# statsleelab/gauss

Measured on AMD Instinct MI355X. Metric: imputed SNPs/sec (whole node) at 1/2/4/8 GPUs; LD-GEMM MFMA TFLOP/s vs peak, higher is better.
Workload: dtype f32

## Files before the change

### gauss_amd/_lib.py

```python
import ctypes as C
import os

import numpy as np

_HERE = os.path.dirname(os.path.abspath(__file__))
LIB_PATH = os.path.join(_HERE, "lib", "libgauss_hip.so")

MODE_POOLED = 0
MODE_WEIGHTED = 1
ST_CLAMPED = 1
ST_NONFINITE = 2
ST_NOCONV = 4
WIN_IMPUTE = 0
WIN_QCAT = 1
WIN_LD = 2
GENO_U8, GENO_2BIT = 0, 1
SLCT_MAX = 32
TRAITS_MORE_MAX = 63
ST_SLCT_SKIPPED = 8
CODE_ADDITIVE, CODE_DOMINANT, CODE_RECESSIVE = 1, 2, 4
GRAM_F32 = 0
GRAM_I8 = 1

_dp = C.POINTER(C.c_double)
_ip = C.POINTER(C.c_int32)
_u8p = C.c_void_p


class WindowDesc(C.Structure):
    _fields_ = [
        ("mode", C.c_int), ("n_pop", C.c_int), ("pop_off", _ip), ("pop_wgt", _dp),
        ("n_measured", C.c_int), ("n_unmeasured", C.c_int),
        ("geno_m", _u8p), ("geno_u", _u8p), ("ld", C.c_int64), ("z1", _dp),
        ("lambda_", C.c_double), ("min_abs_eig", C.c_double),
        ("out_z", _dp), ("out_info", _dp), ("out_status", _ip), ("out_b11", _dp), ("out_b21", _dp),
        ("kind", C.c_int), ("n_head_measured", C.c_int), ("n_pred_measured", C.c_int), ("eig_cutoff", C.c_double),
        ("out_r", _dp), ("out_num_eig", _ip), ("u_codings", C.c_int),
        ("geno_format", C.c_int), ("rows_m", _ip), ("rows_u", _ip), ("pop_src_off", _ip),
        ("slct_max", C.c_int), ("slct_chi2_stop", C.c_double), ("slct_min_var_frac", C.c_double),
        ("slct_forced", _ip), ("n_slct_forced", C.c_int), ("out_slct_n", _ip), ("out_slct_idx", _ip),
        ("out_slct_zin", _dp), ("out_slct_joint", _dp), ("out_slct_zc", _dp), ("out_slct_var", _dp),
        ("n_traits_more", C.c_int), ("z_more", _dp), ("out_z_more", _dp),
        ("out_loo_z", _dp), ("out_loo_info", _dp), ("out_loo_t", _dp),
    ]


class GaussHipError(RuntimeError):
    pass


_lib = None

SYMBOLS = [
    "gauss_hip_init", "gauss_hip_device_count", "gauss_hip_device_of", "gauss_hip_destroy", "gauss_last_error", "gauss_hip_version", "gauss_hip_set_gram_dtype", "gauss_pinned_alloc", "gauss_pinned_free", "gauss_store_upload", "gauss_store_free", "gauss_pack2bit_device", "gauss_ld", "gauss_ld_per_pop", "gauss_ld_per_pop_pairs",
    "gauss_impute_window", "gauss_gene_ld_batch", "gauss_gram_counts", "gauss_job_create",
    "gauss_ld_rows", "gauss_gene_ld_batch_rows", "gauss_job_run", "gauss_job_fetch", "gauss_job_destroy", "gauss_job_span_ms", "gauss_job_profile",
    "gauss_job_profile_get", "gauss_job_work", "gauss_job_stats", "gauss_synth_device",
    "gauss_store_upload_async", "gauss_store_upload_fd_async", "gauss_store_wait", "gauss_store_alloc", "gauss_store_fill", "gauss_store_fill_fd", "gauss_store_upload_fd", "gauss_hip_context_id", "gauss_hip_add_destroy_hook", "gauss_hip_trim_cache", "gauss_hip_source_hash", "gauss_hip_counters", "gauss_job_counters", "gauss_hip_queues",
    "gauss_pop_weights", "gauss_zmix_normal_eq", "gauss_ld_resampled_rows",
]


def load():
    global _lib
    if _lib is not None:
        return _lib
    if not os.path.exists(LIB_PATH):
        raise GaussHipError(
            f"{LIB_PATH} not found: build it with `python -m gauss_amd.build` "
            "(gauss_amd has no CPU fallback by design)")
    lib = C.CDLL(LIB_PATH)
    for name in SYMBOLS:
        if not hasattr(lib, name):
            raise GaussHipError(f"libgauss_hip.so does not export {name}")
    lib.gauss_last_error.restype = C.c_char_p
    lib.gauss_hip_version.restype = C.c_char_p
    lib.gauss_hip_source_hash.restype = C.c_char_p
    lib.gauss_hip_init.argtypes = [C.c_int, C.POINTER(C.c_void_p)]
    lib.gauss_hip_device_count.argtypes = [C.POINTER(C.c_int)]
    lib.gauss_hip_device_of.argtypes = [C.c_void_p]
    lib.gauss_hip_destroy.argtypes = [C.c_void_p]
    lib.gauss_hip_destroy.restype = None
    lib.gauss_hip_set_gram_dtype.argtypes = [C.c_void_p, C.c_int]
    lib.gauss_pinned_alloc.argtypes = [C.c_void_p, C.c_int64, C.POINTER(C.c_void_p)]
    lib.gauss_pinned_free.argtypes = [C.c_void_p, C.c_void_p]
    lib.gauss_store_upload.argtypes = [C.c_void_p, C.c_void_p, C.c_int64, C.POINTER(C.c_void_p)]
    lib.gauss_store_free.argtypes = [C.c_void_p, C.c_void_p]
    lib.gauss_store_upload_async.argtypes = [C.c_void_p, C.c_void_p, C.c_int64, C.POINTER(C.c_void_p)]
    lib.gauss_store_wait.argtypes = [C.c_void_p, C.c_void_p, C.c_int64]
    lib.gauss_store_alloc.argtypes = [C.c_void_p, C.c_int64, C.POINTER(C.c_void_p)]
    lib.gauss_store_fill.argtypes = [C.c_void_p, C.c_void_p, C.c_void_p, C.c_int64, C.c_int64]
    lib.gauss_store_fill_fd.argtypes = [C.c_void_p, C.c_void_p, C.c_int, C.c_int64, C.c_int64, C.c_int64]
    lib.gauss_store_upload_fd.argtypes = [C.c_void_p, C.c_int, C.c_int64, C.c_int64, C.POINTER(C.c_void_p)]
    lib.gauss_ld.argtypes = [C.c_void_p, C.c_int, _u8p, C.c_int, C.c_int64, _ip, _dp, C.c_int,
                             C.c_double, _dp]
    lib.gauss_pack2bit_device.argtypes = [C.c_void_p, C.c_void_p, C.c_int64, C.c_void_p, C.c_int64, C.c_int, _ip, C.c_int]
    lib.gauss_ld_per_pop.argtypes = [C.c_void_p, _u8p, C.c_int, C.c_int64, _ip, C.c_int, _dp]
    lib.gauss_ld_per_pop_pairs.argtypes = [C.c_void_p, _u8p, C.c_int, C.c_int64, _ip, C.c_int, _ip, C.c_int, _ip, _ip, C.c_int64, _dp]
    lib.gauss_impute_window.argtypes = [C.c_void_p, C.POINTER(WindowDesc)]
    lib.gauss_gene_ld_batch.argtypes = [C.c_void_p, C.c_int, _u8p, C.c_int, C.c_int64, _ip, _dp,
                                        C.c_int, _ip, C.c_int, C.c_double, _dp]
    lib.gauss_ld_rows.argtypes = [C.c_void_p, C.c_int, _u8p, C.c_int64, C.c_int, _ip, C.c_int, _ip, _ip, _dp, C.c_int, C.c_double,
                                  C.c_int, _dp]
    lib.gauss_gene_ld_batch_rows.argtypes = [C.c_void_p, C.c_int, _u8p, C.c_int64, C.c_int, _ip, C.c_int, _ip, _ip, _dp, C.c_int,
                                             _ip, C.c_int, C.c_double, C.c_int, _dp]
    lib.gauss_gram_counts.argtypes = [C.c_void_p, _u8p, C.c_int, C.c_int, C.c_int64,
                                      C.POINTER(C.c_int64)]
    lib.gauss_job_create.argtypes = [C.c_void_p, C.POINTER(WindowDesc), C.c_int, C.c_int,
                                     C.POINTER(C.c_void_p)]
    lib.gauss_job_run.argtypes = [C.c_void_p]
    lib.gauss_job_fetch.argtypes = [C.c_void_p]
    lib.gauss_job_destroy.argtypes = [C.c_void_p]
    lib.gauss_job_destroy.restype = None
    lib.gauss_job_span_ms.argtypes = [C.c_void_p, C.c_void_p, _dp]
    lib.gauss_job_profile.argtypes = [C.c_void_p, C.c_int]
    lib.gauss_job_profile_get.argtypes = [C.c_void_p, C.c_int, _dp, C.POINTER(C.c_int64)]
    lib.gauss_job_counters.argtypes = [C.c_void_p, C.POINTER(C.c_int64)]
    lib.gauss_job_work.argtypes = [C.c_void_p, _dp, _dp, _dp, C.POINTER(C.c_int64)]
    lib.gauss_job_stats.argtypes = [C.c_void_p, _dp]
    lib.gauss_hip_context_id.argtypes = [C.c_void_p]
    lib.gauss_hip_context_id.restype = C.c_uint64
    lib.gauss_hip_trim_cache.argtypes = [C.c_void_p, C.POINTER(C.c_int64)]
    lib.gauss_hip_counters.argtypes = [C.c_void_p, C.POINTER(C.c_int64)]
    lib.gauss_hip_queues.argtypes = [C.c_void_p, C.POINTER(C.c_int32)]
    lib.gauss_synth_device.argtypes = [C.c_void_p, C.c_void_p, C.c_int, C.c_int64, _ip, C.c_int,
                                       C.POINTER(C.c_float), C.POINTER(C.c_float), C.c_uint64]
    lib.gauss_pop_weights.argtypes = [C.c_void_p, _dp, C.POINTER(C.c_int64), C.c_int, C.c_int, C.c_double, _dp, _ip]
    lib.gauss_zmix_normal_eq.argtypes = [C.c_void_p, _u8p, C.c_int, C.c_int64, _ip, C.c_int, _ip, C.c_int, _dp, _dp, _dp, _dp,
                                         C.POINTER(C.c_int64)]
    lib.gauss_ld_resampled_rows.argtypes = [C.c_void_p, _u8p, C.c_int64, C.c_int, _ip, C.c_int, _ip, _ip, C.c_int, _ip, _ip, C.c_int64,
                                            C.c_int64, C.c_double, C.c_int, _dp]
    _lib = lib
    return lib


def check(rc):
    if rc != 0:
        raise GaussHipError(f"gauss_hip error {rc}: {load().gauss_last_error().decode()}")


def as_u8(g):
    g = np.ascontiguousarray(g)
    if g.dtype != np.uint8:
        g = g.astype(np.uint8)
    return g


def ptr(a, t):
    return a.ctypes.data_as(t) if a is not None else None
```

### gauss_amd/csrc/gauss_abi.cpp

```cpp
#include "gauss_job.h"

#define JOB_ALIVE(job)                                                                                          \
    do {                                                                                                        \
        if (!(job)) return fail(GAUSS_E_INVALID, "job is NULL");                                                \
        if (!(job)->ctx) return fail(GAUSS_E_INVALID, "the job's context has been destroyed (gauss_hip_destroy)"); \
    } while (0)

static WinSpec spec_from_desc(const gauss_window_desc& d)
{
    WinSpec w;
    w.mode = d.mode; w.n_pop = d.n_pop; w.pop_off = d.pop_off; w.pop_wgt = d.pop_wgt;
    w.M = d.n_measured; w.U = d.n_unmeasured; w.geno_m = d.geno_m; w.geno_u = d.geno_u; w.ld = d.ld;
    w.z1 = d.z1; w.lambda = d.lambda; w.eps = d.min_abs_eig; w.diag = 1.0; w.ld_only = 0;
    w.gene_off = nullptr; w.n_gene = 0;
    w.kind = d.kind; w.n_head = d.n_head_measured; w.n_predm = d.n_pred_measured; w.eig_cutoff = d.eig_cutoff;
    w.u_codings = d.u_codings;
    w.geno_fmt = d.geno_format; w.rows_m = d.rows_m; w.rows_u = d.rows_u; w.pop_src_off = d.pop_src_off;
    w.out_b11 = d.out_b11; w.out_b21 = d.out_b21;
    w.out_loo_z = d.out_loo_z; w.out_loo_info = d.out_loo_info; w.out_loo_t = d.out_loo_t;
    w.n_traits_more = d.n_traits_more; w.z_more = d.z_more; w.out_z_more = d.out_z_more;
    w.slct_max = d.slct_max; w.slct_chi2_stop = d.slct_chi2_stop; w.slct_min_var_frac = d.slct_min_var_frac;
    w.slct_forced = d.slct_forced; w.n_slct_forced = d.n_slct_forced;
    w.out_slct_n = d.out_slct_n; w.out_slct_idx = d.out_slct_idx; w.out_slct_zin = d.out_slct_zin;
    w.out_slct_joint = d.out_slct_joint; w.out_slct_zc = d.out_slct_zc; w.out_slct_var = d.out_slct_var;
// ... 2 lines not shown
extern "C" {

int gauss_job_create(gauss_ctx* ctx, const gauss_window_desc* wins, int n_win, int on_device, gauss_job** out_job)
{
    if (!ctx || !wins || n_win < 1 || !out_job) return fail(GAUSS_E_INVALID, "bad arguments to gauss_job_create");
    std::vector<WinSpec> specs;
    for (int i = 0; i < n_win; i++) {
        if (wins[i].n_unmeasured < 1 && wins[i].kind != GAUSS_WIN_LD &&
            !(wins[i].kind == GAUSS_WIN_QCAT && wins[i].n_pred_measured > 0))
            return fail(GAUSS_E_INVALID, "window %d has no unmeasured SNPs", i);
        specs.push_back(spec_from_desc(wins[i]));
    }
    gauss_job* job = nullptr;
    int rc = job_build(ctx, specs, on_device, &job);
    if (rc) return rc;
    for (int i = 0; i < n_win; i++) {
        Plan& pl = job->plans[i];
        pl.out_z = wins[i].out_z; pl.out_info = wins[i].out_info; pl.out_status = wins[i].out_status;
        pl.out_b11 = wins[i].out_b11; pl.out_b21 = wins[i].out_b21;
        pl.out_r = wins[i].out_r; pl.out_num_eig = wins[i].out_num_eig;
    }
    *out_job = job;
    return GAUSS_OK;
}

int gauss_job_run(gauss_job* job) { JOB_ALIVE(job); return job_run(job, true); }
int gauss_job_fetch(gauss_job* job) { JOB_ALIVE(job); return job_fetch(job); }
void gauss_job_destroy(gauss_job* job) { job_free(job); }

int gauss_job_span_ms(gauss_job* first, gauss_job* last, double* out_ms)
{
    JOB_ALIVE(first); JOB_ALIVE(last);
    if (!out_ms || !first->ran || !last->ran) return fail(GAUSS_E_INVALID, "gauss_job_span_ms: both jobs must have run");
    HIPCHK(hipEventSynchronize(last->done));
    float ms = 0.f;
    HIPCHK(hipEventElapsedTime(&ms, first->begin, last->done));
    *out_ms = (double)ms;
    return GAUSS_OK;
}

int gauss_job_profile(gauss_job* job, int enable)
{
    JOB_ALIVE(job);
    if (job->prof && !enable) prof_collect(job);
    job->prof = enable != 0;
    if (enable) { for (int k = 0; k < 5; k++) { job->prof_ms[k] = 0; job->prof_n[k] = 0; } }
    return GAUSS_OK;
}

int gauss_job_profile_get(gauss_job* job, int kernel, double* out_ms, int64_t* out_launches)
{
    JOB_ALIVE(job);
    if (kernel < 0 || kernel > 4) return fail(GAUSS_E_INVALID, "bad arguments");
    hipStreamSynchronize(job->ctx->stream);
    prof_collect(job);
    if (out_ms) *out_ms = job->prof_ms[kernel];
    if (out_launches) *out_launches = job->prof_n[kernel];
    return GAUSS_OK;
}

int gauss_job_work(gauss_job* job, double* out_ld_flops, double* out_solve_flops, double* out_bytes, int64_t* out_imputed)
{
    if (!job) return fail(GAUSS_E_INVALID, "job is NULL");
    double ldf = 0, sf = 0, by = 0;
    int64_t imp = 0;
    for (const Plan& pl : job->plans) {
        const double M = pl.p.M, U = pl.p.U, N = pl.p.N;
        ldf += N * M * (M + 1) + 2.0 * N * U * M;
        sf += M * M * M / 3.0 + 2.0 * U * M * M + 4.0 * U * M;
        by += (M + U) * N + (M * M + U * M) * 8.0;
        imp += pl.p.U;
    }
    if (out_ld_flops) *out_ld_flops = ldf;
    if (out_solve_flops) *out_solve_flops = sf;
    if (out_bytes) *out_bytes = by;
    if (out_imputed) *out_imputed = imp;
    return GAUSS_OK;
}

int gauss_job_counters(gauss_job* job, int64_t* out4)
{
    if (!job || !out4) return fail(GAUSS_E_INVALID, "bad arguments to gauss_job_counters");
    out4[0] = job->n_merged; out4[1] = job->n_demoted; out4[2] = job->n_giveups; out4[3] = job->n_rerun_failed;
    return GAUSS_OK;
}

int gauss_job_stats(gauss_job* job, double* out4)
{
    if (!job || !out4) return fail(GAUSS_E_INVALID, "bad arguments");
    double flops = 0, slab = 0;
    const bool shm = job->gplan != nullptr;
    const bool edge16 = true;
    auto add = [&](const Plan& pl, bool skip_b11) {
        const Prob& p = pl.p;
        const int mt = p.Mp / TILE;
        auto rows = [&](int t) {
            if (!pl.tile_live.empty()) return pl.tile_live[(size_t)t];
            int left = (t < mt) ? p.M - t * TILE : p.U - (t - mt) * TILE; return left > TILE ? TILE : left;
        };
        auto halves = [](int r, int w) { int n = (r - w * 64 + 31) / 32; return n < 0 ? 0 : (n > 2 ? 2 : n); };
        double k_main = 0;
        {
            const int gran = job->gram_i8 ? 32 : 8;
            const std::vector<int>& blk = (p.geno_fmt == GAUSS_GENO_2BIT && !pl.run_pk_off.empty()) ? pl.run_pk_off : pl.pop_pk_off;
            const bool runs = &blk == &pl.run_pk_off;
            for (size_t q = 0; q + 1 < blk.size(); q++) {
                int live = blk[q + 1] - blk[q];
                if (!runs && q + 1 < pl.pop_raw_off.size()) live = pl.pop_raw_off[q + 1] - pl.pop_raw_off[q];
                else if (runs && pl.run_len_known(q)) live = pl.run_len[q];
                k_main += (double)((live + gran - 1) / gran * gran);
            }
        }
        const bool packed = job->gram_packed && p.slab16;
        int pairs = 0;
        for (int pr = 0; pr < p.npair; pr++) {
            const int ti = pl.pair_ti[pr], tj = pl.pair_tj[pr];
            if (skip_b11 && ti < mt) continue;
            pairs++;
            double tiles32 = 0, tiles_edge = 0;
            for (int wr = 0; wr < 2; wr++)
                for (int wc = 0; wc < 2; wc++) {
                    if (ti == tj && wr == 1 && wc == 0) continue;
                    int na = halves(rows(ti), wr);
                    if (packed && na > 1) na = 1;
                    int nb16 = (rows(tj) - wc * 64 + 15) / 16;
                    nb16 = nb16 < 0 ? 0 : (nb16 > 4 ? 4 : nb16);
                    if (edge16 && !job->gram_i8 && na > 0 && (nb16 & 1)) { tiles_edge += na * nb16 * 0.5; continue; }
                    double t32 = na * halves(rows(tj), wc);
                    if (ti == tj && wr == wc && t32 == 4) t32 = 3;
                    tiles32 += t32;
                }
            flops += 32.0 * 32.0 * 2.0 * (tiles32 * k_main + tiles_edge * p.Kp);
        }
        slab += (double)pairs * p.nseg * TILE * TILE * (p.slab16 ? sizeof(uint16_t) : sizeof(float));
    };
    for (const Plan& pl : job->plans) add(pl, shm);
    if (shm) add(*job->gplan, false);
    out4[0] = job->n_items; out4[1] = flops; out4[2] = slab; out4[3] = (double)job->ws_bytes;
    return GAUSS_OK;
}

int gauss_impute_window(gauss_ctx* ctx, const gauss_window_desc* win)
{
    if (!ctx || !win) return fail(GAUSS_E_INVALID, "bad arguments to gauss_impute_window");
    const bool fused = env_int("GAUSS_FUSED_SOLVE", 1) != 0;
    bool streamed = env_int("GAUSS_STREAM_WINDOW", 1) != 0 && fused && !win->rows_m && !win->rows_u && win->n_unmeasured >= 1 &&
                    win->n_measured >= 1 && win->kind != GAUSS_WIN_LD && (win->u_codings & ~GAUSS_CODE_ADDITIVE) == 0 &&
                    win->geno_m && win->geno_u && win->pop_off && win->n_pop >= 1 && win->n_pop <= 64;
    size_t row_bytes = 0;
    if (streamed) {
        const int N = win->pop_off[win->n_pop];
        if (win->geno_format == GAUSS_GENO_U8) {
            streamed = N >= 1 && win->ld >= N;
            row_bytes = (size_t)std::max(N, 0);
        } else if (win->geno_format == GAUSS_GENO_2BIT && win->ld % 16 == 0) {
            long long end = 0;
            for (int q = 0; q < win->n_pop && streamed; q++) {
                const long long blk = (long long)rup((size_t)std::max(win->pop_off[q + 1] - win->pop_off[q], 0), 64) / 4;
                const long long off = win->pop_src_off ? win->pop_src_off[q] : end;
                if (off < 0 || off % 16 || off + blk > win->ld) streamed = false;
                if (!win->pop_src_off) end = off + blk;
                row_bytes = std::max(row_bytes, (size_t)(off + blk));
            }
        } else streamed = false;
    }
    gauss_job* job = nullptr;
// ... 382 lines not shown
```

### gauss_amd/csrc/gauss_ctx.cpp

```cpp
#include "gauss_job.h"

thread_local std::string g_err;

int fail(int code, const char* fmt, ...)
{
    char buf[512];
    va_list ap;
    va_start(ap, fmt);
    vsnprintf(buf, sizeof(buf), fmt, ap);
    va_end(ap);
    g_err = buf;
    return code;
}

bool trace_on(const char* what)
{
    const char* e = getenv("GAUSS_TRACE");
    if (!e || !*e) return false;
    return strstr(e, "all") != nullptr || strstr(e, what) != nullptr;
}

static std::mutex g_hook_mu;
static std::vector<std::pair<void (*)(gauss_ctx*, uint64_t, void*), void*>> g_destroy_hooks;
static std::atomic<uint64_t> g_next_ctx_id{1};
// ... 105 lines not shown
static void ctx_flush_dev_cache_locked(gauss_ctx* c)
{
    for (auto& kv : c->dev_cache.free_blocks) { (void)hipFree(kv.second); c->block_size.erase(kv.second); }
    c->dev_cache.free_blocks.clear(); c->dev_cache.held = 0;
    (void)hipGetLastError();
}
hipError_t ctx_malloc_retry(gauss_ctx* c, void** out, size_t bytes)
{
    hipError_t e = hipMalloc(out, bytes);
    if (e == hipSuccess) return e;
    {
        std::lock_guard<std::mutex> lock(c->mu);
        if (c->dev_cache.free_blocks.empty()) return e;
        ctx_flush_dev_cache_locked(c);
    }
    return hipMalloc(out, bytes);
}

hipError_t ctx_dev_alloc(gauss_ctx* c, size_t bytes, void** out)
{
    std::lock_guard<std::mutex> lock(c->mu);
    if (void* p = c->dev_cache.take(bytes)) { *out = p; return hipSuccess; }
    hipError_t e = hipMalloc(out, bytes);
    if (e != hipSuccess && !c->dev_cache.free_blocks.empty()) {
        ctx_flush_dev_cache_locked(c);
        e = hipMalloc(out, bytes);
    }
    if (e == hipSuccess) c->block_size[*out] = bytes;
    return e;
}
void ctx_dev_release(gauss_ctx* c, void* p)
{
    if (!p) return;
    std::lock_guard<std::mutex> lock(c->mu);
    auto it = c->block_size.find(p);
    const size_t bytes = it == c->block_size.end() ? 0 : it->second;
    if (bytes && c->dev_cache.held + bytes <= c->dev_cache_limit) { c->dev_cache.free_blocks.emplace(bytes, p); c->dev_cache.held += bytes; return; }
    if (it != c->block_size.end()) c->block_size.erase(it);
    (void)hipFree(p);
}
hipError_t ctx_pin_alloc(gauss_ctx* c, size_t bytes, void** out)
{
    std::lock_guard<std::mutex> lock(c->mu);
    if (void* p = c->pin_cache.take(bytes)) { *out = p; return hipSuccess; }
    hipError_t e = hipHostMalloc(out, bytes, hipHostMallocDefault);
    if (e == hipSuccess) c->block_size[*out] = bytes;
    return e;
}
void ctx_pin_release(gauss_ctx* c, void* p)
{
    if (!p) return;
    std::lock_guard<std::mutex> lock(c->mu);
    auto it = c->block_size.find(p);
    const size_t bytes = it == c->block_size.end() ? 0 : it->second;
    if (bytes && c->pin_cache.held + bytes <= PIN_CACHE_LIMIT) { c->pin_cache.free_blocks.emplace(bytes, p); c->pin_cache.held += bytes; return; }
    if (it != c->block_size.end()) c->block_size.erase(it);
    (void)hipHostFree(p);
}

extern "C" {

const char* gauss_last_error(void) { return g_err.c_str(); }
const char* gauss_hip_version(void) { return "gauss_hip 0.2 (gfx950)"; }

int gauss_hip_init(int device, gauss_ctx** out_ctx)
{
    if (!out_ctx) return fail(GAUSS_E_INVALID, "out_ctx is NULL");
    int n = 0;
    HIPCHK(hipGetDeviceCount(&n));
    if (device < 0 || device >= n) return fail(GAUSS_E_INVALID, "device %d out of range (have %d)", device, n);
    HIPCHK(hipSetDevice(device));
    std::unique_ptr<gauss_ctx> guard(new gauss_ctx());
    gauss_ctx* c = guard.get();
    c->device = device;
    c->id = g_next_ctx_id.fetch_add(1);
    {
        size_t free_b = 0, total_b = 0;
        if (hipMemGetInfo(&free_b, &total_b) != hipSuccess) { total_b = (size_t)288 << 30; (void)hipGetLastError(); }
        c->dev_cache_limit = total_b / 3;
    }
    const char* e = getenv("GAUSS_GRAM_DTYPE");
    c->gram_i8 = (e && (strcmp(e, "i8") == 0 || strcmp(e, "int8") == 0)) ? 1 : 0;
    c->gram_packed = env_int("GAUSS_GRAM_PACKED", 1) != 0 ? 1 : 0;
    const char* one = getenv("GAUSS_SIDE_STREAM");
    c->main_cls = (one && atoi(one) == 0) ? STREAM_NORMAL : STREAM_HIGH;
    int rc = ctx_stream_create(c, &c->stream, c->main_cls);
    if (!rc && c->main_cls == STREAM_HIGH) {
        rc = ctx_stream_create(c, &c->side, STREAM_LOW);
        if (!rc) rc = ctx_stream_create(c, &c->chain, STREAM_HIGH);
    }
    if (!rc) rc = ctx_stream_create(c, &c->upload, STREAM_HIGH);
    if (rc) {
        ctx_stream_destroy(c, &c->upload, STREAM_HIGH);
        ctx_stream_destroy(c, &c->chain, STREAM_HIGH);
        ctx_stream_destroy(c, &c->side, STREAM_LOW);
        ctx_stream_destroy(c, &c->stream, c->main_cls);
        return rc;
    }
    if (c->chain && c->side) c->queues_probed_distinct = queues_side_by_side(c, c->chain, c->stream) && queues_side_by_side(c, c->side, c->stream);
    c->prepin = std::thread([c]() {
        (void)hipSetDevice(c->device);
        {
            void* d = nullptr;
            if (hipMalloc(&d, 256) == hipSuccess) {
                (void)hipMemsetAsync(d, 0, 256, c->upload);
                (void)hipStreamSynchronize(c->upload);
                (void)hipFree(d);
            } else (void)hipGetLastError();
        }
        for (int b = 0; b < 2; b++) {
            void* p = nullptr;
            if (hipHostMalloc(&p, UPLOAD_CHUNK, hipHostMallocDefault) != hipSuccess) { (void)hipGetLastError(); break; }
            { std::lock_guard<std::mutex> lock(c->mu); c->block_size[p] = UPLOAD_CHUNK; }
            ctx_pin_release(c, p);
        }
    });
    { QueueRegistry& r = registry(); std::lock_guard<std::mutex> lock(r.count_mu); r.ctxs.push_back(c); }
    *out_ctx = guard.release();
    return GAUSS_OK;
}

int gauss_hip_device_count(int* out_n)
{
    if (!out_n) return fail(GAUSS_E_INVALID, "out_n is NULL");
    int n = 0;
    hipError_t e = hipGetDeviceCount(&n);
    if (e == hipErrorNoDevice) { n = 0; e = hipSuccess; (void)hipGetLastError(); }
    if (e != hipSuccess) return fail(GAUSS_E_DEVICE, "hipGetDeviceCount failed: %s", hipGetErrorString(e));
    *out_n = n;
    return GAUSS_OK;
}

int gauss_hip_device_of(const gauss_ctx* ctx) { return ctx ? ctx->device : fail(GAUSS_E_INVALID, "ctx is NULL"); }


void gauss_hip_destroy(gauss_ctx* ctx)
{
    if (!ctx) return;
    hipSetDevice(ctx->device);
    ctx_join_prepin(ctx);
    std::vector<std::pair<void (*)(gauss_ctx*, uint64_t, void*), void*>> hooks;
    { std::lock_guard<std::mutex> lock(g_hook_mu); hooks = g_destroy_hooks; }
    for (auto& h : hooks) h.first(ctx, ctx->id, h.second);
    std::vector<gauss_job*> live;
    { std::lock_guard<std::mutex> lock(ctx->mu); live.assign(ctx->jobs.begin(), ctx->jobs.end()); }
    for (gauss_job* j : live) job_release(j);
    hipStreamSynchronize(ctx->stream);
    {
        QueueRegistry& r = registry();
        std::unique_lock<std::shared_mutex> excl(r.mu);
        { std::lock_guard<std::mutex> lock(r.count_mu); r.ctxs.erase(std::remove(r.ctxs.begin(), r.ctxs.end(), ctx), r.ctxs.end()); }
        ctx_stream_destroy(ctx, &ctx->side, STREAM_LOW);
        delete ctx->worker;
        ctx_stream_destroy(ctx, &ctx->copy, STREAM_NORMAL);
        ctx_stream_destroy(ctx, &ctx->aux, STREAM_HIGH);
        ctx_stream_destroy(ctx, &ctx->chain, STREAM_HIGH);
    }
    for (hipEvent_t e : ctx->ev_pool) hipEventDestroy(e);
    if (ctx->landing) (void)hipFree(ctx->landing);
    for (auto& kv : ctx->uploads) kv.second->finish();
    ctx->uploads.clear();
    ctx_stream_destroy(ctx, &ctx->upload, STREAM_HIGH);
    for (auto& kv : ctx->stores) (void)hipFree(const_cast<void*>(kv.first));
    ctx->stores.clear();
    for (auto& kv : ctx->dev_cache.free_blocks) (void)hipFree(kv.second);
    for (auto& kv : ctx->pin_cache.free_blocks) (void)hipHostFree(kv.second);
// ... 78 lines not shown
```

### gauss_amd/csrc/gauss_internal.h

```cpp
#pragma once
#include <hip/hip_runtime.h>
#include <stdint.h>
#include <atomic>
#include <mutex>

namespace gauss {

constexpr int TILE = 128;
constexpr int KC = 64;
constexpr int SEG_MAX = 2048;
constexpr int NB = 64;
constexpr int NR = 64;
constexpr int NRU = NR - 1;
constexpr int WIN_QCAT = 1;
constexpr int WIN_LD = 2;
constexpr int TILE_GB11 = 1 << 30;

#if defined(__HIP_DEVICE_COMPILE__)
#define GP(T) T __attribute__((address_space(1)))*
#else
#define GP(T) T*
#endif

struct Prob {
    int mode, P;
    int M, U;
    int Mp, Up, Sp;
    int N;
    int Kp;
    int nseg, npair, nT;
    int Mld, nblk;
    int npanel;
    int npi;
    int Up128;
    int ld_only;
    int kind;
    int n_head, n_predm;
    int n_rhs;
    int U_raw;
    int code_blk[3];
    int n_run;
    int geno_fmt;
    int gram_i8;
    int slab16;
    double lambda, eps, diag;
    long long ld_raw;
    GP(const uint8_t) raw_m;
    GP(const uint8_t) raw_u;
    GP(uint8_t) packed;
    GP(uint8_t) packed_u;
    GP(int) sx;
    GP(int) sxx;
    GP(int) sx_u;
    GP(int) sxx_u;
    GP(const int) pop_raw_off;
    GP(const int) pop_pk_off;
    GP(const double) pop_w;
    GP(const double) pop_wf;
    GP(const double) pop_md;
    GP(const int) seg_pop;
    GP(const int) seg_k0;
    GP(const int) seg_k1;
    GP(const int) pop_seg0;
    GP(const int) pair_ti;
    GP(const int) pair_tj;
    GP(const int) pair_lut;
    GP(const uint8_t) word_pop;
    GP(const int) rows_m;
    GP(const int) rows_u;
    GP(const uint8_t) word_run;
    GP(const int) run_pk_off;
    GP(const int) run_src;
    GP(float) slab;
    GP(double) rt_sd;
    GP(double) rt_wm;
    GP(double) rt_mu;
    GP(double) rt_wmu;
    GP(double) rt_sd_u;
    GP(double) rt_wm_u;
    GP(double) rt_mu_u;
    GP(double) rt_wmu_u;
    int g0;
    int n_gpair;
    GP(const int) gpair_ti;
    GP(const int) gpair_tj;
    GP(float) slab_g;
    GP(const double) z1;
    GP(double) A;
    GP(double) Linv;
    GP(double) B21;
    GP(double) V;
    GP(double) Gsum;
    GP(double) Part;
    GP(double) out_z;
    GP(double) out_info;
    GP(int) status;
    GP(double) out_ld;
    GP(const int) gene_off;
    int n_gene;
    GP(long long) gene_out_off;
    GP(const int) draw_col;
    int row_src_bytes;
    GP(double) out_loo;
    int slct_max, n_slct_forced;
    double slct_chi2_stop, slct_min_var_frac;
    GP(const int) slct_forced;
    GP(double) slct_W;
    GP(double) out_slct;
    int traits_T;
    GP(const double) traits_Z;
    GP(double) traits_Y;
    GP(double) traits_G;
    GP(double) out_traits;
};
constexpr int TRAITS_MAX = 63;
constexpr int traits_t16(int T) { return (T + 15) & ~15; }
constexpr int SLCT_K = 32;
constexpr int SLCT_T = 512;
constexpr int SLCT_M_MAX = 64 * SLCT_T;
constexpr size_t slct_doubles(int M, int K) { return 2 * (size_t)M + 3 * (size_t)K + 2; }

struct Item {
    GP(const uint8_t) a;
    GP(const uint8_t) b;
    GP(float) slab;
    GP(const int) seg_k1;
    GP(const uint32_t) chunk_live;
    int Kp;
    int k0;
    int nseg;
    int rows_a, rows_b;
    int flags;
};
static_assert(sizeof(Item) == 64, "work items are fetched as one 64-byte descriptor");

template <typename T> using gptr = T __attribute__((address_space(1)))*;
template <typename T> __device__ __forceinline__ gptr<T> G(T* p) { return (gptr<T>)p; }
template <typename T> __device__ __forceinline__ gptr<T> G(gptr<T> p) { return p; }

#if defined(__HIPCC__)
template <typename T>
__device__ __forceinline__ T uniform_load(GP(const T) p, int idx)
{
    return ((const T __attribute__((address_space(4)))*)p)[idx];
}
__device__ __forceinline__ int chunk_live_units(uint32_t word, int chunk)
{
    const int n = (int)((word >> (4 * (chunk & 7))) & 15u);
    return n ? n : 8;
}
#endif

struct DeviceOnce {
    std::atomic<unsigned long long> done{0};
    std::mutex mu;
    template <typename F> void run(F&& set)
    {
        int d = 0;
        (void)hipGetDevice(&d);
        const unsigned long long bit = 1ull << (d & 63);
        if (done.load(std::memory_order_acquire) & bit) return;
        std::lock_guard<std::mutex> lock(mu);
        if (done.load(std::memory_order_relaxed) & bit) return;
        set();
        done.fetch_or(bit, std::memory_order_release);
    }
};

void launch_pack_stats(const Prob* d_probs, const int2* d_rowmap, int n_rows, hipStream_t s);
constexpr int SIMLD_LDS_MAX = 60 << 10;
int resample_pack_lds_bytes(long long row_src_bytes);
void launch_resample_pack(const Prob* d_probs, const int2* d_rowmap, int n_rows, int lds_bytes, hipStream_t s);
void launch_gram(const Item* d_items, int n_items, int dtype_i8, hipStream_t s, unsigned long long* d_b11_done = nullptr);
void launch_wait_count(const unsigned long long* d_count, unsigned long long target, int* d_status, int n_status, hipStream_t s,
                       double bound_us = 0.0);
void launch_wait_count_for(const unsigned long long* d_count, unsigned long long target, int* d_status, hipStream_t s, double bound_us);
void launch_count_up(unsigned long long* d_count, hipStream_t s);
void launch_epilogue(const Prob* d_probs, const int2* d_tilemap, int n_tiles, int max_pop, int dtype_i8, hipStream_t s);
void launch_epilogue_b11_lite(const Prob* d_probs, const int2* d_tilemap, int n_tiles, int dtype_i8, hipStream_t s);
void launch_pop_cor(const Prob* d_probs, int prob, int npair, double* d_out, hipStream_t s);
void launch_zmix_normal_eq(const Prob* d_probs, int prob, int npair, const int* d_pop_group, int n_group, const double* d_z,
                           double* d_part, long long* d_part_n, double* d_out, long long* d_out_n, hipStream_t s);
void launch_pair_cor(const Prob* d_probs, int prob, const int2* d_pairs, long long n_pairs, const int* d_pop_group, int n_group,
                     double* d_out, hipStream_t s);
void launch_gene_epilogue(const Prob* d_probs, int prob, int n_gene, hipStream_t s);
void launch_factor_step(const Prob* d_probs, int n_prob, int step, int max_nblk, int max_npanel, int split, int own_panel, hipStream_t s);
void launch_factor_step_lite(const Prob* d_probs, int n_prob, int step, int max_nblk, int max_npanel, int split, hipStream_t s);
void launch_solve_last_lite(const Prob* d_probs, const int2* d_panelmap, int n_panels, int max_nblk, int split, hipStream_t s);
void launch_shift_cert(const Prob* d_probs, int n_prob, hipStream_t s);
void launch_solve(const Prob* d_probs, const int2* d_panelmap, int n_panels, hipStream_t s);
void launch_impute_gemm(const Prob* d_probs, const int2* d_gmap, int n_tiles, int u_tile, const int2* d_fmap, int n_chunks, hipStream_t s);
void launch_solve_last(const Prob* d_probs, const int2* d_panelmap, int n_panels, int max_nblk, int split, hipStream_t s);
void launch_loo(const Prob* d_probs, const int2* d_loomap, int n_panels, hipStream_t s);
void launch_slct(const Prob* d_probs, const int* d_slctmap, int n, hipStream_t s);
void launch_traits_weights(const Prob* d_probs, const int2* d_map, int n_blocks, hipStream_t s);
void launch_traits_impute(const Prob* d_probs, const int2* d_umap, int n_strips, hipStream_t s);
void launch_counts(const Prob* d_probs, int prob, int npair, long long* d_out, hipStream_t s);
void launch_pack2bit(const uint8_t* d_in, long long ld_in, uint8_t* d_out, long long ld_out, int n_snp,
                     const int* d_pop_off, const int* d_blk_off, int n_pop, hipStream_t s);
void launch_h2d_copy(void* d_dst, const void* pinned_src, size_t bytes, hipStream_t s);
struct ExportD {
    const double* src;
    double* dst;
    int rows, width, pitch, pad_;
};
void launch_export_rows(const ExportD* d_exports, int n, long long max_elems, hipStream_t s);
struct PwChunk { long long r0, r1; int iv, pad_; };
void launch_pop_weights(const double* d_x, int n_pop, const PwChunk* d_chunks, int n_chunk, const int* d_chunk_off,
                        const long long* d_off, int n_interval, double eps, double* d_part1, double* d_mean, double* d_part2,
                        double* d_w, int* d_status, hipStream_t s);
void launch_synth(uint8_t* d_out, int n_snp, long long ld, const int* d_pop_off, int n_pop,
                  int n_samples, const float* d_thr, const float* d_rho, uint64_t seed,
                  hipStream_t s);

}
```

### gauss_amd/csrc/gauss_job.h

```cpp
#pragma once
#include "gauss_internal.h"
#pragma GCC visibility push(default)
#include "../../include/gauss_hip.h"
#pragma GCC visibility pop

#include <algorithm>
#include <atomic>
#include <chrono>
#include <condition_variable>
#include <cmath>
#include <cstdarg>
#include <cstdio>
#include <cstring>
#include <deque>
#include <functional>
#include <map>
#include <memory>
#include <mutex>
#include <set>
#include <shared_mutex>
#include <thread>
#include <string>
#include <vector>

// ... 33 lines not shown

struct CopyWorker {
    std::mutex mu;
    std::condition_variable cv;
    std::function<void()> task;
    bool busy = false, stop = false;
    std::thread th;
    explicit CopyWorker(int device)
    {
        th = std::thread([this, device]() {
            (void)hipSetDevice(device);
            std::unique_lock<std::mutex> lock(mu);
            for (;;) {
                cv.wait(lock, [&] { return stop || task; });
                if (stop) return;
                std::function<void()> t;
                t.swap(task);
                lock.unlock();
                t();
                lock.lock();
                busy = false;
                cv.notify_all();
            }
        });
    }
    void submit(std::function<void()> t)
    {
        std::lock_guard<std::mutex> lock(mu);
        task = std::move(t); busy = true;
        cv.notify_all();
    }
    void wait()
    {
        std::unique_lock<std::mutex> lock(mu);
        cv.wait(lock, [&] { return !busy; });
    }
    ~CopyWorker()
    {
        { std::lock_guard<std::mutex> lock(mu); stop = true; cv.notify_all(); }
        if (th.joinable()) th.join();
    }
};

struct StoreUpload {
    void* d = nullptr;
    size_t bytes = 0;
    std::thread th;
    std::mutex mu;
    std::condition_variable cv;
    std::vector<std::pair<size_t, hipEvent_t>> marks;
    bool done = false;
    int rc = 0;
    std::string err;
    std::mutex join_mu;
    void finish() { std::lock_guard<std::mutex> lock(join_mu); if (th.joinable()) th.join(); }
    ~StoreUpload()
    {
        finish();
        for (auto& m : marks) if (m.second) hipEventDestroy(m.second);
    }
};

enum StreamClass { STREAM_NORMAL = 0, STREAM_HIGH = 1, STREAM_LOW = 2 };

struct gauss_ctx {
    int device;
    uint64_t id = 0;
    hipStream_t stream = nullptr;
    StreamClass main_cls = STREAM_HIGH;
    hipStream_t side = nullptr;
    hipStream_t copy = nullptr;
    hipStream_t aux = nullptr;
    hipStream_t chain = nullptr;
    struct CopyWorker* worker = nullptr;
    uint8_t* landing = nullptr;
    size_t landing_bytes = 0;
    std::vector<hipEvent_t> ev_pool;
    std::mutex stream_mu;
    std::mutex run_mu;
    hipStream_t upload = nullptr;
    std::map<const void*, std::shared_ptr<StoreUpload>> uploads;
    int gram_i8 = 0;
    int gram_packed = 1;
    std::map<const void*, size_t> stores;
    std::mutex mu;
    BlockCache dev_cache, pin_cache;
    std::map<void*, size_t> block_size;
    std::set<gauss_job*> jobs;
    size_t dev_cache_limit = 0;
    std::thread prepin;
    std::mutex prepin_mu;
    int n_hi = 0, n_lo = 0;
    bool queues_probed_distinct = false;
    std::atomic<long long> n_runs_merged{0}, n_runs_demoted{0}, n_merged_giveups{0}, n_rerun_failed{0};
};

int ctx_stream_create(gauss_ctx* c, hipStream_t* out, StreamClass cls);
void ctx_stream_destroy(gauss_ctx* c, hipStream_t* s, StreamClass cls);
std::shared_mutex& queue_registry_mutex();
bool queues_exclusive(int device);
void ctx_join_prepin(gauss_ctx* c);

hipError_t ctx_malloc_retry(gauss_ctx* c, void** out, size_t bytes);
hipError_t ctx_dev_alloc(gauss_ctx* c, size_t bytes, void** out);
void ctx_dev_release(gauss_ctx* c, void* p);
hipError_t ctx_pin_alloc(gauss_ctx* c, size_t bytes, void** out);
void ctx_pin_release(gauss_ctx* c, void* p);

bool trace_on(const char* what);

constexpr double GRAM_PACKED_COST = 0.58;
static inline int env_int(const char* name, int dflt) { const char* e = getenv(name); return e ? atoi(e) : dflt; }

constexpr int GEMM_SMALL_TILES = 1600;
constexpr int OWN_PANEL_MAX_WINDOWS = 20;
constexpr int SOLVE_SPLIT_MIN = 2;

static const size_t PIN_CACHE_LIMIT = (size_t)1 << 30;
static const size_t UPLOAD_CHUNK = (size_t)32 << 20;
static inline size_t rup(size_t x, size_t a) { return (x + a - 1) / a * a; }

struct DevBuf {
    void* p = nullptr;
    DevBuf() = default;
    DevBuf(const DevBuf&) = delete;
    DevBuf& operator=(const DevBuf&) = delete;
    ~DevBuf() { if (p) (void)hipFree(p); }
    hipError_t alloc(size_t bytes) { return hipMalloc(&p, bytes ? bytes : 1); }
    hipError_t alloc(gauss_ctx* c, size_t bytes) { return ctx_malloc_retry(c, &p, bytes ? bytes : 1); }
    template <typename T> T* as() const { return (T*)p; }
};
struct Plan {
    Prob p;
    std::vector<int> pop_raw_off, pop_pk_off, seg_pop, seg_k0, seg_k1, pop_seg0;
    std::vector<int> pair_ti, pair_tj, pair_lut;
    std::vector<double> pop_w, pop_wf, pop_md, z1;
    std::vector<uint8_t> word_pop, word_run;
    std::vector<uint32_t> chunk_live;
    std::vector<int> run_pk_off, run_src, run_len;
    bool run_len_known(size_t q) const { return q < run_len.size(); }
    std::vector<int32_t> rows_m, rows_u;
    std::vector<int32_t> draw_col;
    size_t row_bytes = 0;
    std::vector<int> gene_off;
    std::vector<long long> gene_out_off;
    std::vector<std::pair<int, int>> groups;
    std::vector<std::pair<int, int>> fine;
    std::vector<int> tile_live;
    const uint8_t* h_geno_m = nullptr;
    const uint8_t* h_geno_u = nullptr;
    long long user_ld = 0;
    double* out_z = nullptr;
    double* out_info = nullptr;
    int32_t* out_status = nullptr;
    double* out_b11 = nullptr;
    double* out_b21 = nullptr;
    double* out_r = nullptr;
    int32_t* out_num_eig = nullptr;
    bool loo = false;
    double* out_loo_z = nullptr;
    double* out_loo_info = nullptr;
    double* out_loo_t = nullptr;
    int slct_K = 0;
    std::vector<int> slct_forced;
    int32_t* out_slct_n = nullptr;
    int32_t* out_slct_idx = nullptr;
    double* out_slct_zin = nullptr;
    double* out_slct_joint = nullptr;
    double* out_slct_zc = nullptr;
    double* out_slct_var = nullptr;
    int traits_T = 0;
    std::vector<double> traits_z;
    double* out_z_more = nullptr;
    size_t res_count() const
    { return 2 * (size_t)p.n_rhs + (loo ? 3 * (size_t)p.M : 0) + (size_t)traits_T * p.U + (slct_K ? slct_doubles(p.M, slct_K) : 0); }
    double* out_ld_user = nullptr;
    int U_user = 0;
    size_t out_ld_count = 0;
    double* d_b11_copy = nullptr;
    size_t res_off = 0;
};

struct ProfSlot { hipEvent_t a, b; int kernel; unsigned run; int launches = 1; };

struct gauss_job {
    gauss_ctx* ctx = nullptr;
    int n = 0;
    int on_device = 0;
    std::vector<Plan> plans;
    char* d_tab = nullptr;      size_t tab_bytes = 0;
    char* d_ws = nullptr;       size_t ws_bytes = 0;
    std::vector<char> h_tab;
    char* h_pin = nullptr;
    hipEvent_t begin = nullptr;
    hipEvent_t zeroed = nullptr;
    hipEvent_t done = nullptr;
    struct RunEvents { hipEvent_t gram = nullptr, side = nullptr, pack = nullptr, rows = nullptr, epi = nullptr; };
    RunEvents rev[2];
    Prob* d_probs = nullptr;
    Item* d_items = nullptr;    int n_items = 0;
    int2* d_rowmap = nullptr;   int n_rows = 0;
    std::unique_ptr<Plan> gplan;
    std::vector<int> g0;
    std::vector<std::vector<int2>> win_tiles;
    int2* d_tilemap = nullptr;  int n_tiles = 0;
    int n_tiles_b11 = 0;
    int n_items_b11 = 0;
    bool chain_aside = false;
    int2* d_panelmap = nullptr; int n_panels = 0;
    int2* d_dpanelmap = nullptr; int n_dpanels = 0;
    int2* d_gemmmap = nullptr;  int n_gemm = 0;
    int gemm_ut = 128;
    int2* d_finmap = nullptr;   int n_fin = 0;
    int* d_slctmap = nullptr;   int n_slct = 0;
    int2* d_traitsmap = nullptr;  int n_traits = 0;
    int2* d_traitsumap = nullptr; int n_traits_u = 0;
    int2* d_loomap = nullptr;   int n_loo = 0;
    int max_nblk = 0;
    int max_npanel = 0;
    int solve_split = 0;
    int own_panel = 0;
    struct StreamGroup { int item0, n_items, row0, n_rows, tile0, n_tiles; };
    std::vector<StreamGroup> sgroups;
    std::vector<hipEvent_t> sevp;
    int max_pop = 1;
    int gram_i8 = 0;
    int gram_packed = 0;
    int resample_lds = -1;
    int* d_status = nullptr;
    unsigned long long* d_b11_done = nullptr;
    bool merged = false;
    bool force_merged = false;
    bool queue_touched = false;
    hipStream_t zero_queue = nullptr;
    double wait_bound_us = 0.0;
    unsigned long long merged_runs = 0;
    int n_items_b21_early = 0;
    int n_tiles_b21_early = 0;
    double* d_results = nullptr; size_t n_results = 0;
    double* h_res2[2] = {nullptr, nullptr};
    int* h_st2[2] = {nullptr, nullptr};
    hipEvent_t done2[2] = {nullptr, nullptr};
    unsigned run_seq = 0, fetch_seq = 0;
    double* h_results = nullptr;
    int* h_status = nullptr;
    struct Export { int plan, which; size_t off; int rows, width, pitch; double* user; };
    std::vector<Export> exports;
    std::vector<std::pair<int, int>> exp_chunks;
    std::vector<hipEvent_t> exp_ev;
    double* h_export = nullptr;
    ExportD* d_exports = nullptr;
    bool prof = false;
    std::vector<ProfSlot> slots;
    double prof_ms[5] = {0, 0, 0, 0, 0};
    long long prof_n[5] = {0, 0, 0, 0, 0};
    bool ran = false;
    bool ran_solve = true;
    unsigned prof_run = 0;
    long long n_merged = 0, n_demoted = 0, n_giveups = 0, n_rerun_failed = 0;
};

struct StreamSetup {
    uint8_t* d_m = nullptr;
    uint8_t* d_u = nullptr;
    long long ldraw = 0;
    size_t row_bytes = 0;
    int M = 0, U = 0;
    std::vector<int> first_tile;
    std::vector<int> tile_group;
    std::vector<hipEvent_t> ev;
    std::mutex mu;
    std::condition_variable cv;
    int recorded = 0, rc = 0;
    std::string err;
    int n_groups() const { return (int)first_tile.size() - 1; }
};

struct WinSpec {
    int mode, n_pop;
    const int32_t* pop_off;
    const double* pop_wgt;
    int M, U;
    const uint8_t* geno_m;
    const uint8_t* geno_u;
    long long ld;
    const double* z1;
    double lambda, eps, diag;
    int ld_only;
    const int32_t* gene_off;
    int n_gene;
    int kind = 0, n_head = 0, n_predm = 0;
    int u_codings = 0;
    int geno_fmt = 0;
    const int32_t* rows_m = nullptr;
    const int32_t* rows_u = nullptr;
    const int32_t* pop_src_off = nullptr;
    double eig_cutoff = 0.01;
    const int32_t* pair_i = nullptr;
    const int32_t* pair_j = nullptr;
    int64_t n_pairs = 0;
    int gram_only = 0;
    double* out_b11 = nullptr;
    double* out_b21 = nullptr;
    double* out_loo_z = nullptr;
    double* out_loo_info = nullptr;
    double* out_loo_t = nullptr;
    int n_traits_more = 0;
    const double* z_more = nullptr;
    double* out_z_more = nullptr;
    int slct_max = 0;
// ... 26 lines not shown
```

### gauss_amd/csrc/gauss_plan.cpp

```cpp
#include "gauss_job.h"

static int seg_max_for(const std::vector<WinSpec>& specs)
{
    if (specs.size() >= 4) return 4096;
    double pairs = 0, kp = 0;
    for (const WinSpec& w : specs) {
        if (w.gene_off || w.pair_i || w.M < 1 || w.n_pop < 1 || w.n_pop > 64 || !w.pop_off) return SEG_MAX;
        int nc = 0;
        for (int c = 0; c < 3; c++) nc += (w.u_codings >> c) & 1;
        const double mt = (w.M + TILE - 1) / TILE, ut = ((double)w.U * std::max(nc, 1) + TILE - 1) / TILE;
        pairs += mt * (mt + 1) / 2 + ut * mt;
        kp = std::max(kp, w.draw_pop ? (double)w.n_drawn + 32.0 : (double)w.pop_off[w.n_pop] + 32.0 * w.n_pop);
    }
    const double want = pairs * kp / 1300.0;
    return (int)std::min<double>(SEG_MAX, std::max<double>(384.0, std::floor(want / KC) * KC));
}
static int group_target_for(size_t n_windows)
{
    return n_windows >= 4 ? 2048 : 0;
}
int plan_problem(const WinSpec& w, Plan& pl, int seg_max, int group_target)
{
    if (w.mode != GAUSS_MODE_POOLED && w.mode != GAUSS_MODE_WEIGHTED) return fail(GAUSS_E_INVALID, "bad mode %d", w.mode);
    if (w.n_pop < 1 || w.n_pop > 64) return fail(GAUSS_E_INVALID, "n_pop must be in 1..64 (got %d)", w.n_pop);
// ... 219 lines not shown
        long long off = 0;
        for (int g = 0; g < w.n_gene; g++) {
            const int r0 = pl.gene_off[g], r1 = pl.gene_off[g + 1];
            if (r0 < 0 || r1 < r0 || r1 > w.M) return fail(GAUSS_E_INVALID, "gene_off out of range at gene %d", g);
            pl.gene_out_off.push_back(off);
            off += (long long)(r1 - r0) * (r1 - r0);
            if (r1 > r0)
                for (int ti = r0 / TILE; ti <= (r1 - 1) / TILE; ti++)
                    for (int tj = ti; tj <= (r1 - 1) / TILE; tj++) add_pair(ti, tj);
        }
        pl.out_ld_count = (size_t)off;
        p.n_gene = w.n_gene;
    } else if (w.pair_i) {
        for (int64_t k = 0; k < w.n_pairs; k++) {
            const int i = w.pair_i[k], j = w.pair_j[k];
            if (i < 0 || j <= i || j >= w.M) return fail(GAUSS_E_INVALID, "pair %lld = (%d, %d) is not i < j < n_snp", (long long)k, i, j);
            add_pair(i / TILE, j / TILE);
        }
        pl.out_ld_count = 0;
    } else {
        for (int ti = 0; ti < mt; ti++)
            for (int tj = ti; tj < mt; tj++) add_pair(ti, tj);
        for (int tu = mt; tu < p.nT; tu++)
            for (int tj = 0; tj < mt; tj++) add_pair(tu, tj);
        if (w.ld_only && !w.gram_only) pl.out_ld_count = (size_t)w.M * w.M;
    }
    p.npair = (int)pl.pair_ti.size();
    p.Mld = (int)rup((size_t)w.M, NB);
    p.nblk = p.Mld / NB;
    p.npanel = (w.ld_only || w.kind == GAUSS_WIN_LD) ? 0 : (p.n_rhs + NRU - 1) / NRU;
    p.npi = p.npanel > 0 ? (w.M + 1 + NR - 1) / NR : 0;
    p.Up128 = (int)rup((size_t)std::max(p.n_rhs, 1), 128);
    pl.U_user = w.U;
    if (w.z1) pl.z1.assign(w.z1, w.z1 + w.M);
    pl.h_geno_m = w.geno_m; pl.h_geno_u = w.geno_u; pl.user_ld = w.ld;
    pl.out_b11 = w.out_b11; pl.out_b21 = w.out_b21;
    pl.loo = loo; pl.out_loo_z = w.out_loo_z; pl.out_loo_info = w.out_loo_info; pl.out_loo_t = w.out_loo_t;
    pl.slct_K = w.slct_max;
    pl.slct_forced.clear();
    if (w.slct_max > 0) {
        pl.slct_forced.assign(w.slct_forced, w.slct_forced + w.n_slct_forced);
        p.slct_max = w.slct_max; p.n_slct_forced = w.n_slct_forced;
        p.slct_chi2_stop = w.slct_chi2_stop; p.slct_min_var_frac = w.slct_min_var_frac;
    }
    pl.traits_T = w.n_traits_more; pl.out_z_more = w.out_z_more;
    pl.traits_z.clear();
    if (w.n_traits_more > 0) {
        const int T16 = traits_t16(w.n_traits_more);
        pl.traits_z.assign((size_t)p.Mld * T16, 0.0);
        for (int t = 0; t < w.n_traits_more; t++)
            for (int g = 0; g < w.M; g++) pl.traits_z[(size_t)g * T16 + t] = w.z_more[(size_t)t * w.M + g];
        p.traits_T = w.n_traits_more;
    }
    pl.out_slct_n = w.out_slct_n; pl.out_slct_idx = w.out_slct_idx; pl.out_slct_zin = w.out_slct_zin;
    pl.out_slct_joint = w.out_slct_joint; pl.out_slct_zc = w.out_slct_zc; pl.out_slct_var = w.out_slct_var;
    return GAUSS_OK;
}

struct Arena {
    size_t off = 0;
    size_t take(size_t bytes) { size_t o = off; off = rup(off + bytes, 256); return o; }
};

template <typename T>
static size_t put(std::vector<char>& blob, Arena& a, const std::vector<T>& v)
{
    const size_t bytes = std::max<size_t>(v.size() * sizeof(T), 1);
    const size_t o = a.take(bytes);
    if (blob.size() < a.off) blob.resize(a.off);
    if (!v.empty()) memcpy(blob.data() + o, v.data(), v.size() * sizeof(T));
    return o;
}
int job_build(gauss_ctx* ctx, const std::vector<WinSpec>& specs, int on_device, gauss_job** out, const StreamSetup* stream)
{
    const bool streamed = stream != nullptr;
    const auto tb0 = std::chrono::steady_clock::now();
    gauss_job* job = new gauss_job();
    std::unique_ptr<gauss_job, void (*)(gauss_job*)> guard(job, job_free);
    job->ctx = ctx;
    job->n = (int)specs.size();
    job->on_device = on_device;
    job->gram_i8 = ctx->gram_i8;
    job->gram_packed = (ctx->gram_packed && !ctx->gram_i8) ? 1 : 0;
    job->plans.resize(job->n);
    for (const WinSpec& w : specs)
        if (w.draw_pop && (specs.size() != 1 || streamed)) return fail(GAUSS_E_INVALID, "a resampled window is a job of its own");
    const int seg_max = seg_max_for(specs);
    for (int i = 0; i < job->n; i++) {
        int rc = plan_problem(specs[i], job->plans[i], seg_max, group_target_for(specs.size()));
        if (rc) return rc;
        job->plans[i].p.gram_i8 = job->gram_i8;
        if (!job->plans[i].draw_col.empty()) job->resample_lds = resample_pack_lds_bytes(job->plans[i].p.row_src_bytes);
    }
    size_t exp_doubles = 0;
    if (!streamed) {
        for (int i = 0; i < job->n; i++) {
            const Plan& pl = job->plans[i];
            const Prob& p = pl.p;
            const bool has = p.kind == GAUSS_WIN_LD || p.npanel > 0;
            if (!has) continue;
            if (pl.out_b11) { job->exports.push_back(gauss_job::Export{i, 0, exp_doubles, p.M, p.M, p.Mld, pl.out_b11}); exp_doubles += (size_t)p.M * p.M; }
            if (pl.out_b21 && p.U > 0) { job->exports.push_back(gauss_job::Export{i, 1, exp_doubles, p.U, p.M, p.Mld, pl.out_b21}); exp_doubles += (size_t)p.U * p.M; }
            exp_doubles = rup(exp_doubles, 32);
        }
        if (exp_doubles * sizeof(double) > ((size_t)256 << 20)) { job->exports.clear(); exp_doubles = 0; }
    }
    const auto tb1 = std::chrono::steady_clock::now();
    if (on_device && !streamed && job->n >= 2 && env_int("GAUSS_SHARE_MEASURED", 1) != 0) {
        const Plan& a = job->plans[0];
        bool ok = true;
        std::vector<int32_t> gl;
        std::vector<int> g0((size_t)job->n, 0);
        std::set<std::pair<int, int>> have;
        size_t cl0 = 0, own_pairs = 0;
        for (int i = 0; i < job->n && ok; i++) {
            const Plan& b = job->plans[i];
            ok = !b.rows_m.empty() && !b.p.ld_only && !b.p.n_gene && b.p.P <= 32 && b.h_geno_m == a.h_geno_m && b.user_ld == a.user_ld &&
                 b.p.mode == a.p.mode && b.p.P == a.p.P && b.p.geno_fmt == a.p.geno_fmt && b.p.slab16 == a.p.slab16 && b.p.Kp == a.p.Kp &&
                 b.pop_raw_off == a.pop_raw_off && b.pop_pk_off == a.pop_pk_off && b.pop_w == a.pop_w && b.seg_k0 == a.seg_k0 &&
                 b.seg_k1 == a.seg_k1 && b.seg_pop == a.seg_pop && b.run_src == a.run_src && b.run_pk_off == a.run_pk_off &&
                 b.groups == a.groups;
            if (!ok) break;
            const size_t M = b.rows_m.size(), mt = (M + TILE - 1) / TILE;
            own_pairs += mt * (mt + 1) / 2;
            size_t pos = gl.size();
            bool join = false;
            if (gl.size() > cl0 && std::is_sorted(gl.begin() + (ptrdiff_t)cl0, gl.end())) {
                const int32_t first = b.rows_m[0];
                const size_t p0 = (size_t)(std::lower_bound(gl.begin() + (ptrdiff_t)cl0, gl.end(), first) - gl.begin());
                if (p0 < gl.size() && gl[p0] == first) {
                    join = true;
                    for (size_t k = 0; k < M && join; k++) {
                        if (k > 0 && b.rows_m[k] <= b.rows_m[k - 1]) join = false;
                        else if (p0 + k < gl.size() && gl[p0 + k] != b.rows_m[k]) join = false;
                    }
                    if (join) {
                        const int lo = (int)(p0 / TILE), hi = (int)((p0 + M - 1) / TILE);
                        size_t add = 0;
                        for (int ti = lo; ti <= hi; ti++)
                            for (int tj = ti; tj <= hi; tj++) add += have.count(std::make_pair(ti, tj)) ? 0 : 1;
                        join = add <= mt * (mt + 1) / 2;
                        pos = p0;
                    }
                }
            }
            if (!join) {
                gl.resize(rup(gl.size(), TILE), -1);
                cl0 = pos = gl.size();
            }
            g0[(size_t)i] = (int)pos;
            for (size_t k = 0; k < M; k++)
                if (pos + k >= gl.size()) gl.push_back(b.rows_m[k]);
            const int lo = (int)(pos / TILE), hi = (int)((pos + M - 1) / TILE);
            for (int ti = lo; ti <= hi; ti++)
                for (int tj = ti; tj <= hi; tj++) have.insert(std::make_pair(ti, tj));
        }
        if (ok && (long long)gl.size() < (1 << 24) && (have.size() < own_pairs || env_int("GAUSS_SHARE_MEASURED", 1) == 2)) {
            job->gplan.reset(new Plan(a));
            job->g0 = g0;
            Plan& g = *job->gplan;
            g.rows_m = gl;
            g.rows_u.clear(); g.z1.clear(); g.gene_off.clear(); g.gene_out_off.clear();
            Prob& q = g.p;
            q.M = (int)gl.size(); q.U = 0; q.U_raw = 1; q.n_rhs = 0;
            q.Mp = (int)rup((size_t)q.M, TILE); q.Up = 0; q.Sp = q.Mp; q.nT = q.Mp / TILE;
            q.Mld = 0; q.nblk = 0; q.npanel = 0; q.npi = 0; q.kind = 0; q.ld_only = 0; q.n_head = q.n_predm = 0;
// ... 312 lines not shown
    const size_t o_traitsumap = traitsumap.empty() ? 0 : put(blob, ta, traitsumap);
    const size_t o_probs = ta.take(sizeof(Prob) * (size_t)n_prob);
    const size_t o_exports = ta.take(sizeof(ExportD) * std::max<size_t>(job->exports.size(), 1));
    blob.resize(ta.off);
    job->n_items = (int)items.size();
    job->n_rows = (int)rowmap.size();
    job->n_tiles = (int)tilemap.size();
    job->n_panels = (int)panelmap.size();
    job->n_dpanels = (int)dpanelmap.size();
    job->n_gemm = (int)gemmmap.size();
    job->n_fin = (int)finmap.size();
    job->n_loo = (int)loomap.size();
    job->n_slct = (int)slctmap.size();
    job->n_traits = (int)traitsmap.size();
    job->n_traits_u = (int)traitsumap.size();

    Arena wa;
    Arena wslab;
    struct WsOff { size_t raw_m, raw_u, packed, sx, sxx, slab, sd, wm, mu, wmu, A, Linv, B21, V, ld, b11c, gsum, part, slct, ty, tg; long long ldraw; };
    std::vector<WsOff> wo(job->n);
    size_t res = 0;
    {
        int n_solve = 0;
        for (int i = 0; i < job->n; i++) n_solve += job->plans[i].p.npanel > 0 ? 1 : 0;
        job->own_panel = (n_solve > 0 && n_solve <= OWN_PANEL_MAX_WINDOWS) ? 1 : 0;
        job->solve_split = job->n_panels > 0 ? SOLVE_SPLIT_MIN : 0;
    }
    for (int i = 0; i < job->n; i++) {
        Plan& pl = job->plans[i];
        Prob& p = pl.p;
        WsOff& w = wo[i];
        if (streamed) {
            w.ldraw = stream->ldraw;
        } else if (!on_device) {
            const bool linear = pl.rows_m.empty() && pl.rows_u.empty() && (size_t)pl.user_ld <= pl.row_bytes + pl.row_bytes / 8 + 64;
            w.ldraw = linear ? pl.user_ld : (long long)rup(pl.row_bytes, 16);
            w.raw_m = wa.take((size_t)p.M * w.ldraw + 64);
            w.raw_u = wa.take((size_t)std::max(pl.U_user, 1) * w.ldraw + 64);
        } else {
            w.ldraw = pl.user_ld;
        }
        w.packed = wa.take((size_t)p.Sp * p.Kp);
        w.sx = wa.take((size_t)p.Sp * p.P * sizeof(int));
        w.sxx = wa.take((size_t)p.Sp * p.P * sizeof(int));
        w.slab = wslab.take((size_t)p.npair * p.nseg * TILE * TILE * (p.slab16 ? sizeof(uint16_t) : sizeof(float)));
        w.sd = wa.take((size_t)p.Sp * sizeof(double));
        w.wm = wa.take((size_t)p.Sp * sizeof(double));
        w.mu = wa.take((size_t)p.Sp * p.P * sizeof(double));
        w.wmu = wa.take((size_t)p.Sp * p.P * sizeof(double));
        if (!p.ld_only) {
            w.A = wa.take((size_t)(p.npanel > 0 ? 5 : 2) * p.Mld * p.Mld * sizeof(double));
            w.B21 = wa.take((size_t)std::max(p.U, 1) * p.Mld * sizeof(double));
        }
        if (p.npanel > 0) {
            w.Linv = wa.take((size_t)2 * p.nblk * NB * NB * sizeof(double));
            w.V = wa.take((size_t)std::max(p.npanel, p.npi) * p.Mld * NR * sizeof(double));
            w.gsum = wa.take((size_t)((p.Mld + 127) / 128) * p.Up128 * 3 * sizeof(double));
            w.part = wa.take((size_t)2 * p.npi * 4 * NB * NR * sizeof(double));
            w.b11c = wa.take((size_t)p.Mld * p.Mld * sizeof(double));
        }
        w.slct = pl.slct_K ? wa.take((size_t)SLCT_K * p.Mld * sizeof(double)) : 0;
        w.ty = w.tg = 0;
        if (pl.traits_T) {
            w.ty = wa.take((size_t)p.Mld * traits_t16(pl.traits_T) * sizeof(double));
            w.tg = wa.take((size_t)p.Mld * traits_t16(pl.traits_T) * sizeof(double));
        }
        w.ld = wa.take(std::max<size_t>(pl.out_ld_count, 1) * sizeof(double));
        pl.res_off = res;
        res += pl.res_count();
    }
    struct GOff { size_t packed, sx, sxx, sd, wm, mu, wmu, slab; } go = {0, 0, 0, 0, 0, 0, 0, 0};
    if (shm) {
        const Prob& q = job->gplan->p;
        const size_t rows = (size_t)q.Mp + TILE;
        go.packed = wa.take(rows * q.Kp);
        go.sx = wa.take(rows * q.P * sizeof(int));
        go.sxx = wa.take(rows * q.P * sizeof(int));
        go.sd = wa.take(rows * sizeof(double));
        go.wm = wa.take(rows * sizeof(double));
        go.mu = wa.take(rows * q.P * sizeof(double));
        go.wmu = wa.take(rows * q.P * sizeof(double));
        go.slab = wslab.take((size_t)q.npair * q.nseg * TILE * TILE * (q.slab16 ? sizeof(uint16_t) : sizeof(float)));
    }
    const size_t o_status = wa.take(sizeof(int) * (4 * job->n + 4));
    const size_t o_count = wa.take(128);
    const size_t o_results = wa.take(sizeof(double) * std::max<size_t>(res, 1));
    job->n_results = res;
    const size_t slab_base = rup(wa.off, 4096);
    for (WsOff& w : wo) w.slab += slab_base;
    go.slab += slab_base;
    job->ws_bytes = slab_base + wslab.off;
    job->tab_bytes = rup(blob.size(), 16);

    const bool job_trace = trace_on("job");
    const auto tj0 = std::chrono::steady_clock::now();
    hipError_t e = ctx_dev_alloc(ctx, job->ws_bytes, (void**)&job->d_ws);
    if (e != hipSuccess) { job->d_ws = nullptr; return fail(GAUSS_E_NOMEM, "hipMalloc(%zu bytes workspace) failed: %s", wa.off, hipGetErrorString(e)); }
    e = ctx_dev_alloc(ctx, job->tab_bytes, (void**)&job->d_tab);
    if (e != hipSuccess) { job->d_tab = nullptr; return fail(GAUSS_E_NOMEM, "hipMalloc(%zu bytes tables) failed", blob.size()); }
    const size_t pin_tab = rup(job->tab_bytes, 256), pin_res = rup(sizeof(double) * std::max<size_t>(res, 1), 256);
    const size_t pin_st = rup(sizeof(int) * (4 * job->n + 4), 256);
    const size_t pin_exp = rup(sizeof(double) * exp_doubles, 256);
    e = ctx_pin_alloc(ctx, pin_tab + 2 * (pin_res + pin_st) + pin_exp, (void**)&job->h_pin);
    if (e != hipSuccess) { job->h_pin = nullptr; return fail(GAUSS_E_NOMEM, "hipHostMalloc(%zu bytes) failed", pin_tab + 2 * pin_res); }
    for (int k = 0; k < 2; k++) {
        job->h_res2[k] = (double*)(job->h_pin + pin_tab + k * (pin_res + pin_st));
        job->h_st2[k] = (int*)(job->h_pin + pin_tab + k * (pin_res + pin_st) + pin_res);
        HIPCHK(hipEventCreate(&job->done2[k]));
    }
    job->h_results = job->h_res2[0];
    job->h_status = job->h_st2[0];
    job->done = job->done2[0];
    if (!job->exports.empty()) {
        job->h_export = (double*)(job->h_pin + pin_tab + 2 * (pin_res + pin_st));
        const size_t per = std::max<size_t>((size_t)1 << 18, (exp_doubles + 31) / 32);
        size_t acc = 0;
        int first = 0;
        const int nx = (int)job->exports.size();
        for (int x = 0; x < nx; x++) {
            acc += (size_t)job->exports[(size_t)x].rows * job->exports[(size_t)x].width;
            if (acc >= per || x + 1 == nx) { job->exp_chunks.push_back(std::make_pair(first, x + 1)); first = x + 1; acc = 0; }
        }
        job->exp_ev.assign(job->exp_chunks.size(), nullptr);
        for (hipEvent_t& ev : job->exp_ev) HIPCHK(hipEventCreateWithFlags(&ev, hipEventDisableTiming));
    }
    const auto tj1 = std::chrono::steady_clock::now();
    HIPCHK(hipEventCreate(&job->begin));
    for (int k = 0; k < 2; k++)
        for (hipEvent_t* e : {&job->rev[k].gram, &job->rev[k].side, &job->rev[k].pack, &job->rev[k].rows, &job->rev[k].epi})
            HIPCHK(hipEventCreateWithFlags(e, hipEventDisableTiming));

    hipStream_t st = ctx->stream;
    hipStream_t zs = st;
    {
        std::lock_guard<std::mutex> lock(ctx->mu);
        if (ctx->upload && ctx->uploads.empty()) zs = ctx->upload;
    }
    job->queue_touched = true;
    job->zero_queue = zs;
    HIPCHK(hipMemsetAsync(job->d_ws, 0, slab_base, zs));
    if (zs != st) {
        HIPCHK(hipEventCreateWithFlags(&job->zeroed, hipEventDisableTiming));
        HIPCHK(hipEventRecord(job->zeroed, zs));
        HIPCHK(hipStreamWaitEvent(st, job->zeroed, 0));
    }
    if (streamed) {
        job->sevp.resize(job->sgroups.size(), nullptr);
        for (hipEvent_t& e : job->sevp) HIPCHK(hipEventCreateWithFlags(&e, hipEventDisableTiming));
    }

    job->d_status = (int*)(job->d_ws + o_status);
    job->d_b11_done = (unsigned long long*)(job->d_ws + o_count);
    job->d_results = (double*)(job->d_ws + o_results);
    std::deque<std::vector<uint8_t>> stage;
    for (int i = 0; i < job->n; i++) {
        Plan& pl = job->plans[i];
        Prob& p = pl.p;
        const WsOff& w = wo[i];
        char* T = job->d_tab;
        char* W = job->d_ws;
        p.ld_raw = w.ldraw;
        if (streamed) { p.raw_m = stream->d_m; p.raw_u = stream->d_u; }
        else if (on_device) { p.raw_m = pl.h_geno_m; p.raw_u = pl.h_geno_u; }
        else { p.raw_m = (const uint8_t*)(W + w.raw_m); p.raw_u = (const uint8_t*)(W + w.raw_u); }
        p.packed = (uint8_t*)(W + w.packed);
        p.sx = (int*)(W + w.sx); p.sxx = (int*)(W + w.sxx);
        p.pop_raw_off = (const int*)(T + to[i].raw_off);
        p.pop_pk_off = (const int*)(T + to[i].pk_off);
        p.pop_w = (const double*)(T + to[i].w);
        p.pop_wf = (const double*)(T + to[i].wf);
        p.pop_md = (const double*)(T + to[i].md);
        p.seg_pop = (const int*)(T + to[i].seg_pop);
        p.seg_k0 = (const int*)(T + to[i].k0);
        p.seg_k1 = (const int*)(T + to[i].k1);
        p.pop_seg0 = (const int*)(T + to[i].seg0);
        p.pair_ti = (const int*)(T + to[i].ti);
        p.pair_tj = (const int*)(T + to[i].tj);
        p.pair_lut = (const int*)(T + to[i].lut);
        p.word_pop = (const uint8_t*)(T + to[i].wp);
        p.word_run = (const uint8_t*)(T + to[i].wr);
        p.rows_m = (on_device && !pl.rows_m.empty()) ? (const int*)(T + to[i].rm) : nullptr;
        p.rows_u = (on_device && !pl.rows_u.empty()) ? (const int*)(T + to[i].ru) : nullptr;
        p.run_pk_off = (const int*)(T + to[i].rpk);
        p.run_src = (const int*)(T + to[i].rsrc);
        p.slab = (float*)(W + w.slab);
        p.rt_sd = (double*)(W + w.sd); p.rt_wm = (double*)(W + w.wm);
        p.rt_mu = (double*)(W + w.mu); p.rt_wmu = (double*)(W + w.wmu);
        p.z1 = (const double*)(T + to[i].z1);
        if (!p.ld_only) { p.A = (double*)(W + w.A); p.B21 = (double*)(W + w.B21); }
        if (p.npanel > 0) {
            p.Linv = (double*)(W + w.Linv); p.V = (double*)(W + w.V); p.Gsum = (double*)(W + w.gsum);
            p.Part = (double*)(W + w.part);
            pl.d_b11_copy = (double*)(W + w.b11c);
        }
        p.out_z = job->d_results + pl.res_off;
        p.out_info = job->d_results + pl.res_off + p.n_rhs;
        p.out_loo = pl.loo ? job->d_results + pl.res_off + 2 * (size_t)p.n_rhs : nullptr;
        p.out_slct = pl.slct_K ? job->d_results + pl.res_off + pl.res_count() - slct_doubles(p.M, pl.slct_K) : nullptr;
        p.slct_W = pl.slct_K ? (double*)(W + w.slct) : nullptr;
        p.out_traits = pl.traits_T ? job->d_results + pl.res_off + 2 * (size_t)p.n_rhs + (pl.loo ? 3 * (size_t)p.M : 0) : nullptr;
        p.traits_Z = pl.traits_T ? (const double*)(T + to[i].tz) : nullptr;
        p.traits_Y = pl.traits_T ? (double*)(W + w.ty) : nullptr;
        p.traits_G = pl.traits_T ? (double*)(W + w.tg) : nullptr;
        p.slct_forced = pl.slct_forced.empty() ? nullptr : (const int*)(T + to[i].sf);
        p.status = job->d_status + 4 * i;
        p.out_ld = (double*)(W + w.ld);
        p.gene_off = p.n_gene ? (const int*)(T + to[i].goff) : nullptr;
        p.gene_out_off = p.n_gene ? (long long*)(T + to[i].gout) : nullptr;
        p.draw_col = pl.draw_col.empty() ? nullptr : (const int*)(T + to[i].dc);
        p.packed_u = p.packed + (size_t)p.Mp * p.Kp;
        p.sx_u = p.sx + (size_t)p.Mp * p.P; p.sxx_u = p.sxx + (size_t)p.Mp * p.P;
        p.rt_sd_u = p.rt_sd + p.Mp; p.rt_wm_u = p.rt_wm + p.Mp;
        p.rt_mu_u = p.rt_mu + (size_t)p.Mp * p.P; p.rt_wmu_u = p.rt_wmu + (size_t)p.Mp * p.P;
        p.g0 = 0; p.n_gpair = 0; p.gpair_ti = p.pair_ti; p.gpair_tj = p.pair_tj; p.slab_g = p.slab;
        if (shm) {
            const Prob& q = job->gplan->p;
            const size_t g0 = (size_t)job->g0[(size_t)i];
            p.g0 = (int)g0; p.n_gpair = q.npair;
            p.packed = (uint8_t*)(W + go.packed) + g0 * q.Kp;
            p.sx = (int*)(W + go.sx) + g0 * q.P; p.sxx = (int*)(W + go.sxx) + g0 * q.P;
            p.rt_sd = (double*)(W + go.sd) + g0; p.rt_wm = (double*)(W + go.wm) + g0;
            p.rt_mu = (double*)(W + go.mu) + g0 * q.P; p.rt_wmu = (double*)(W + go.wmu) + g0 * q.P;
            p.gpair_ti = (const int*)(T + to[(size_t)job->n].ti); p.gpair_tj = (const int*)(T + to[(size_t)job->n].tj);
            p.slab_g = (float*)(W + go.slab);
        }
        memcpy(blob.data() + o_probs + sizeof(Prob) * i, &p, sizeof(Prob));
        if (!on_device && !streamed) {
            auto upload = [&](size_t dst_off, const uint8_t* src, const std::vector<int32_t>& rows, int nrows) -> int {
                if (nrows <= 0) return GAUSS_OK;
                if (rows.empty()) {
                    if (w.ldraw == pl.user_ld)
                        HIPCHK(hipMemcpyAsync(W + dst_off, src, (size_t)(nrows - 1) * pl.user_ld + pl.row_bytes,
                                              hipMemcpyHostToDevice, st));
                    else
                        HIPCHK(hipMemcpy2DAsync(W + dst_off, (size_t)w.ldraw, src, (size_t)pl.user_ld, pl.row_bytes,
                                                (size_t)nrows, hipMemcpyHostToDevice, st));
                    return GAUSS_OK;
                }
                stage.emplace_back((size_t)nrows * w.ldraw);
                std::vector<uint8_t>& buf = stage.back();
                for (int r = 0; r < nrows; r++)
                    memcpy(buf.data() + (size_t)r * w.ldraw, src + (size_t)rows[r] * pl.user_ld, pl.row_bytes);
                HIPCHK(hipMemcpyAsync(W + dst_off, buf.data(), buf.size(), hipMemcpyHostToDevice, st));
                return GAUSS_OK;
            };
            int rc = upload(w.raw_m, pl.h_geno_m, pl.rows_m, p.M);
            if (!rc) rc = upload(w.raw_u, pl.h_geno_u, pl.rows_u, pl.U_user);
            if (rc) return rc;
        }
    }
    if (shm) {
        Plan& g = *job->gplan;
        Prob& q = g.p;
        const size_t n = (size_t)job->n;
        char* T = job->d_tab;
        char* W = job->d_ws;
        q.ld_raw = g.user_ld;
        q.raw_m = g.h_geno_m; q.raw_u = nullptr;
        q.packed = (uint8_t*)(W + go.packed); q.packed_u = q.packed;
        q.sx = (int*)(W + go.sx); q.sxx = (int*)(W + go.sxx); q.sx_u = q.sx; q.sxx_u = q.sxx;
        q.rt_sd = (double*)(W + go.sd); q.rt_wm = (double*)(W + go.wm); q.rt_sd_u = q.rt_sd; q.rt_wm_u = q.rt_wm;
        q.rt_mu = (double*)(W + go.mu); q.rt_wmu = (double*)(W + go.wmu); q.rt_mu_u = q.rt_mu; q.rt_wmu_u = q.rt_wmu;
        q.pop_raw_off = (const int*)(T + to[n].raw_off); q.pop_pk_off = (const int*)(T + to[n].pk_off);
        q.pop_w = (const double*)(T + to[n].w); q.pop_wf = (const double*)(T + to[n].wf); q.pop_md = (const double*)(T + to[n].md);
        q.seg_pop = (const int*)(T + to[n].seg_pop); q.seg_k0 = (const int*)(T + to[n].k0); q.seg_k1 = (const int*)(T + to[n].k1);
        q.pop_seg0 = (const int*)(T + to[n].seg0);
        q.pair_ti = (const int*)(T + to[n].ti); q.pair_tj = (const int*)(T + to[n].tj); q.pair_lut = (const int*)(T + to[n].lut);
        q.word_pop = (const uint8_t*)(T + to[n].wp); q.word_run = (const uint8_t*)(T + to[n].wr);
        q.rows_m = (const int*)(T + to[n].rm); q.rows_u = nullptr;
        q.run_pk_off = (const int*)(T + to[n].rpk); q.run_src = (const int*)(T + to[n].rsrc);
        q.slab = (float*)(W + go.slab); q.slab_g = q.slab; q.gpair_ti = q.pair_ti; q.gpair_tj = q.pair_tj; q.g0 = 0; q.n_gpair = q.npair;
        q.z1 = nullptr; q.A = nullptr; q.B21 = nullptr; q.Linv = nullptr; q.V = nullptr; q.Gsum = nullptr; q.Part = nullptr;
        q.out_z = q.out_info = nullptr; q.out_loo = nullptr; q.out_slct = nullptr; q.slct_W = nullptr; q.slct_forced = nullptr; q.slct_max = 0; q.traits_T = 0; q.traits_Z = nullptr; q.traits_Y = q.traits_G = q.out_traits = nullptr; q.out_ld = nullptr; q.status = job->d_status;
        q.gene_off = nullptr; q.gene_out_off = nullptr; q.n_gene = 0;
        memcpy(blob.data() + o_probs + sizeof(Prob) * n, &q, sizeof(Prob));
    }
    for (size_t n = 0; n < items.size(); n++) {
        const ItemH& h = items[n];
        const Plan& pl = plan_of(h.prob);
        const Prob& p = pl.p;
        const std::pair<int, int>& gr = h.group >= 0 ? pl.groups[h.group] : pl.fine[(size_t)(-1 - h.group)];
        const int ti = pl.pair_ti[h.pair], tj = pl.pair_tj[h.pair];
        const int mt = p.Mp / TILE;
        auto rows = [&](int t) {
            if (!pl.tile_live.empty()) return pl.tile_live[(size_t)t];
            int left = (t < mt) ? p.M - t * TILE : p.U - (t - mt) * TILE; return left > TILE ? TILE : left;
        };
        auto tile_rows = [&](int t) { return t < mt ? p.packed + (size_t)t * TILE * p.Kp : p.packed_u + (size_t)(t - mt) * TILE * p.Kp; };
        Item it;
        it.a = tile_rows(ti);
        it.b = tile_rows(tj);
        it.slab = p.slab + ((size_t)h.pair * p.nseg + gr.first) * (p.slab16 ? TILE * TILE / 2 : TILE * TILE);
        it.seg_k1 = p.seg_k1 + gr.first;
        it.chunk_live = (const uint32_t*)(job->d_tab + to[h.prob].ch);
        it.Kp = p.Kp; it.k0 = pl.seg_k0[gr.first]; it.nseg = gr.second - gr.first;
        it.rows_a = rows(ti); it.rows_b = rows(tj); it.flags = (ti == tj ? 1 : 0) | (p.slab16 ? 2 : 0) | (p.slab16 && job->gram_packed ? 4 : 0);
        if (job->merged && (int)n < job->n_items_b11) it.flags |= 16;
        else if (job->merged && (int)n < job->n_items_b11 + job->n_items_b21_early) it.flags |= 32;
        memcpy(blob.data() + o_items + sizeof(Item) * n, &it, sizeof(Item));
    }
    for (size_t x = 0; x < job->exports.size(); x++) {
        const gauss_job::Export& ex = job->exports[x];
        const Plan& pl = job->plans[(size_t)ex.plan];
        ExportD d;
        d.src = ex.which ? pl.p.B21 : (pl.p.kind == GAUSS_WIN_LD ? pl.p.A : pl.d_b11_copy);
        d.dst = job->h_export + ex.off;
        d.rows = ex.rows; d.width = ex.width; d.pitch = ex.pitch; d.pad_ = 0;
        memcpy(blob.data() + o_exports + sizeof(ExportD) * x, &d, sizeof(ExportD));
    }
    const auto tj2 = std::chrono::steady_clock::now();
    memcpy(job->h_pin, blob.data(), blob.size());
    launch_h2d_copy(job->d_tab, job->h_pin, job->tab_bytes, st);
    HIPCHK(hipGetLastError());
    if (job_trace) {
        auto ms = [](std::chrono::steady_clock::time_point a, std::chrono::steady_clock::time_point b) { return std::chrono::duration<double, std::milli>(b - a).count(); };
        fprintf(stderr, "[job] %d windows: plan %.2f ms (the windows' plans %.2f, shared rows + row checks %.2f, tables + work items %.2f), allocations %.2f ms (workspace %.1f MB, tables %.2f MB, pinned %.2f MB), events + zeroing + tables %.2f ms, table copy queued in %.2f ms\n",
                job->n, ms(tb0, tj0), ms(tb0, tb1), ms(tb1, tb2), ms(tb2, tj0), ms(tj0, tj1), job->ws_bytes / 1e6, job->tab_bytes / 1e6, (pin_tab + 2 * (pin_res + pin_st)) / 1e6, ms(tj1, tj2),
                ms(tj2, std::chrono::steady_clock::now()));
    }
    job->d_probs = (Prob*)(job->d_tab + o_probs);
    job->d_items = (Item*)(job->d_tab + o_items);
    job->d_rowmap = (int2*)(job->d_tab + o_rowmap);
    job->d_tilemap = (int2*)(job->d_tab + o_tilemap);
    job->d_panelmap = (int2*)(job->d_tab + o_panelmap);
    job->d_dpanelmap = (int2*)(job->d_tab + o_dpanelmap);
    job->d_gemmmap = (int2*)(job->d_tab + o_gemmmap);
    job->d_finmap = (int2*)(job->d_tab + o_finmap);
    job->d_loomap = (int2*)(job->d_tab + o_loomap);
    job->d_slctmap = (int*)(job->d_tab + o_slctmap);
    job->d_traitsmap = (int2*)(job->d_tab + o_traitsmap);
    job->d_traitsumap = (int2*)(job->d_tab + o_traitsumap);
    job->d_exports = (ExportD*)(job->d_tab + o_exports);
    if (!on_device && !streamed) HIPCHK(hipStreamSynchronize(st));
    std::vector<char>().swap(job->h_tab);
    { std::lock_guard<std::mutex> lock(ctx->mu); ctx->jobs.insert(job); }
    *out = guard.release();
    return GAUSS_OK;
}
```

### gauss_amd/csrc/gauss_run.cpp

```cpp
#include "gauss_job.h"

static void prof_begin(gauss_job* job, int kernel, hipStream_t st, int launches = 1)
{
    if (!job->prof) return;
    ProfSlot s;
    s.kernel = kernel;
    s.launches = launches;
    s.run = job->prof_run;
    hipEventCreate(&s.a);
    hipEventCreate(&s.b);
    hipEventRecord(s.a, st);
    job->slots.push_back(s);
}
static void prof_end(gauss_job* job, hipStream_t st)
{
    if (!job->prof) return;
    hipEventRecord(job->slots.back().b, st);
}
void prof_collect(gauss_job* job, unsigned run_end)
{
    std::vector<ProfSlot> keep;
    for (ProfSlot& s : job->slots) {
        if (run_end != ~0u && (int)(s.run - run_end) >= 0) { keep.push_back(s); continue; }
        hipEventSynchronize(s.b);
        float ms = 0.f;
        hipEventElapsedTime(&ms, s.a, s.b);
        job->prof_ms[s.kernel] += ms;
        job->prof_n[s.kernel] += s.launches;
        hipEventDestroy(s.a);
        hipEventDestroy(s.b);
    }
    job->slots.swap(keep);
}


static int queue_exports(gauss_job* job, size_t c0, size_t c1, hipStream_t st)
{
    for (size_t c = c0; c < c1 && c < job->exp_chunks.size(); c++) {
        const int x0 = job->exp_chunks[c].first, x1 = job->exp_chunks[c].second;
        long long mx = 0;
        for (int x = x0; x < x1; x++) mx = std::max(mx, (long long)job->exports[(size_t)x].rows * job->exports[(size_t)x].width);
        launch_export_rows(job->d_exports + x0, x1 - x0, mx, st);
        HIPCHK(hipEventRecord(job->exp_ev[c], st));
    }
    return GAUSS_OK;
}

static int job_queue_results(gauss_job* job, int par, hipStream_t st)
{
    HIPCHK(hipGetLastError());
    const bool job_trace = trace_on("job");
    const auto t0 = std::chrono::steady_clock::now();
    { const int rc = queue_exports(job, 0, job->exp_chunks.size(), st); if (rc) return rc; }
    if (job->n_results) launch_h2d_copy(job->h_res2[par], job->d_results, rup(sizeof(double) * job->n_results, 16), st);
    launch_h2d_copy(job->h_st2[par], job->d_status, sizeof(int) * (4 * job->n + 4), st);
    HIPCHK(hipGetLastError());
    HIPCHK(hipEventRecord(job->done2[par], st));
    if (job_trace) fprintf(stderr, "[job] run: result copies queued in %.2f ms\n", std::chrono::duration<double, std::milli>(std::chrono::steady_clock::now() - t0).count());
    job->done = job->done2[par];
    return GAUSS_OK;
}

static int job_queue_run(gauss_job* job, bool solve, int par, bool allow_merged)
{
    gauss_ctx* ctx = job->ctx;
    hipStream_t st = ctx->stream;
    const gauss_job::RunEvents& ev = job->rev[par];
    job->queue_touched = true;
    std::lock_guard<std::mutex> run_lock(ctx->run_mu);
    std::shared_lock<std::shared_mutex> qlock(queue_registry_mutex());
    const bool merged = job->merged && allow_merged && solve && (job->force_merged || (ctx->queues_probed_distinct && queues_exclusive(ctx->device)));
    if (job->merged && solve) { (merged ? ctx->n_runs_merged : ctx->n_runs_demoted)++; (merged ? job->n_merged : job->n_demoted)++; }
    const auto t_run0 = std::chrono::steady_clock::now();
    HIPCHK(hipEventRecord(job->begin, st));
    HIPCHK(hipMemsetAsync(job->d_status, 0, sizeof(int) * (4 * job->n + 4), st));
    if (trace_on("job")) fprintf(stderr, "[job] run (%s): begin mark + status zeroing queued in %.2f ms\n", merged ? "merged" : (job->chain_aside ? "two launches" : "one queue"),
                                 std::chrono::duration<double, std::milli>(std::chrono::steady_clock::now() - t_run0).count());
    const bool fused = env_int("GAUSS_FUSED_SOLVE", 1) != 0 || job->n_loo > 0 || job->n_traits > 0;
    hipStream_t side = (solve && fused && job->n_panels > 0 && job->n_tiles > job->n_tiles_b11) ? ctx->side : nullptr;
    prof_begin(job, 1, st);
    if (job->resample_lds >= 0) launch_resample_pack(job->d_probs, job->d_rowmap, job->n_rows, job->resample_lds, st);
    else launch_pack_stats(job->d_probs, job->d_rowmap, job->n_rows, st);
    const bool cert_on_chain = solve && job->chain_aside && merged;
    if (solve && job->n_panels > 0 && !cert_on_chain) launch_shift_cert(job->d_probs, job->n, st);
    prof_end(job, st);
    if (solve && job->chain_aside) {
        hipStream_t ch = ctx->chain;
        if (merged) {
            HIPCHK(hipEventRecord(ev.gram, st));
            prof_begin(job, 0, st, 1);
            launch_gram(job->d_items, job->n_items, job->gram_i8, st, job->d_b11_done);
            job->merged_runs++;
            prof_end(job, st);
            HIPCHK(hipStreamWaitEvent(ch, ev.gram, 0));
            if (cert_on_chain) launch_shift_cert(job->d_probs, job->n, ch);
            launch_wait_count(job->d_b11_done, job->merged_runs * (unsigned long long)job->n_items_b11, job->d_status + 4 * job->n, 1, ch, job->wait_bound_us);
        } else {
            prof_begin(job, 0, st, 2);
            launch_gram(job->d_items, job->n_items_b11, job->gram_i8, st);
            HIPCHK(hipEventRecord(ev.gram, st));
            launch_gram(job->d_items + job->n_items_b11, job->n_items - job->n_items_b11, job->gram_i8, st);
            prof_end(job, st);
            HIPCHK(hipStreamWaitEvent(ch, ev.gram, 0));
        }
        prof_begin(job, 2, ch);
        launch_epilogue_b11_lite(job->d_probs, job->d_tilemap, job->n_tiles_b11, job->gram_i8, ch);
        prof_end(job, ch);
        for (int i = 0; i < job->n; i++) {
            Plan& pl = job->plans[i];
            if (pl.out_b11 && pl.p.npanel > 0)
                HIPCHK(hipMemcpyAsync(pl.d_b11_copy, pl.p.A, sizeof(double) * pl.p.Mld * pl.p.Mld, hipMemcpyDeviceToDevice, ch));
        }
        prof_begin(job, 3, ch);
        for (int s = 0; s < job->max_nblk; s++)
            launch_factor_step_lite(job->d_probs, job->n, s, job->max_nblk, job->max_npanel, job->solve_split, ch);
        launch_solve_last_lite(job->d_probs, job->d_panelmap, job->n_panels, job->max_nblk, job->solve_split, ch);
        prof_end(job, ch);
        HIPCHK(hipEventRecord(ev.side, ch));
        if (merged && job->n_tiles_b21_early > 0) {
            hipStream_t lo = ctx->side;
            HIPCHK(hipStreamWaitEvent(lo, ev.gram, 0));
            launch_wait_count(job->d_b11_done + 8, job->merged_runs * (unsigned long long)job->n_items_b21_early, job->d_status + 4 * job->n, 1, lo, job->wait_bound_us);
            launch_epilogue(job->d_probs, job->d_tilemap + job->n_tiles_b11, job->n_tiles_b21_early, job->max_pop, job->gram_i8, lo);
            HIPCHK(hipEventRecord(ev.epi, lo));
            prof_begin(job, 2, st);
            launch_epilogue(job->d_probs, job->d_tilemap + job->n_tiles_b11 + job->n_tiles_b21_early,
                            job->n_tiles - job->n_tiles_b11 - job->n_tiles_b21_early, job->max_pop, job->gram_i8, st);
            prof_end(job, st);
            HIPCHK(hipStreamWaitEvent(st, ev.epi, 0));
        } else {
            prof_begin(job, 2, st);
            launch_epilogue(job->d_probs, job->d_tilemap + job->n_tiles_b11, job->n_tiles - job->n_tiles_b11, job->max_pop, job->gram_i8, st);
            prof_end(job, st);
        }
        HIPCHK(hipStreamWaitEvent(st, ev.side, 0));
        prof_begin(job, 4, st);
        launch_loo(job->d_probs, job->d_loomap, job->n_loo, st);
        launch_slct(job->d_probs, job->d_slctmap, job->n_slct, st);
        launch_traits_weights(job->d_probs, job->d_traitsmap, job->n_traits, st);
        launch_impute_gemm(job->d_probs, job->d_gemmmap, job->n_gemm, job->gemm_ut, job->d_finmap, job->n_fin, st);
        launch_traits_impute(job->d_probs, job->d_traitsumap, job->n_traits_u, st);
        prof_end(job, st);
        return job_queue_results(job, par, st);
    }
    prof_begin(job, 0, st, 1);
    launch_gram(job->d_items, job->n_items, job->gram_i8, st);
    prof_end(job, st);
    if (side) {
        HIPCHK(hipEventRecord(ev.gram, st));
        HIPCHK(hipStreamWaitEvent(side, ev.gram, 0));
        launch_epilogue(job->d_probs, job->d_tilemap + job->n_tiles_b11, job->n_tiles - job->n_tiles_b11, job->max_pop, job->gram_i8, side);
        HIPCHK(hipEventRecord(ev.side, side));
    }
    prof_begin(job, 2, st);
    launch_epilogue(job->d_probs, job->d_tilemap, side ? job->n_tiles_b11 : job->n_tiles, job->max_pop, job->gram_i8, st);
    for (int i = 0; i < job->n; i++)
        if (job->plans[i].p.n_gene) launch_gene_epilogue(job->d_probs, i, job->plans[i].p.n_gene, st);
    prof_end(job, st);
    if (solve && job->n_panels > 0) {
        for (int i = 0; i < job->n; i++) {
            Plan& pl = job->plans[i];
            if (pl.out_b11 && pl.p.npanel > 0)
                HIPCHK(hipMemcpyAsync(pl.d_b11_copy, pl.p.A, sizeof(double) * pl.p.Mld * pl.p.Mld, hipMemcpyDeviceToDevice, st));
        }
        prof_begin(job, 3, st);
        for (int s = 0; s < job->max_nblk; s++)
            launch_factor_step(job->d_probs, job->n, s, job->max_nblk, fused ? job->max_npanel : 0, job->solve_split,
                               job->own_panel, st);
        prof_end(job, st);
        prof_begin(job, 4, st);
        if (fused) {
            launch_solve_last(job->d_probs, job->d_panelmap, job->n_panels, job->max_nblk, job->solve_split, st);
            if (side) HIPCHK(hipStreamWaitEvent(st, ev.side, 0));
            launch_loo(job->d_probs, job->d_loomap, job->n_loo, st);
            launch_slct(job->d_probs, job->d_slctmap, job->n_slct, st);
            launch_traits_weights(job->d_probs, job->d_traitsmap, job->n_traits, st);
            launch_impute_gemm(job->d_probs, job->d_gemmmap, job->n_gemm, job->gemm_ut, job->d_finmap, job->n_fin, st);
            launch_traits_impute(job->d_probs, job->d_traitsumap, job->n_traits_u, st);
        } else {
            launch_slct(job->d_probs, job->d_slctmap, job->n_slct, st);
            launch_solve(job->d_probs, job->d_dpanelmap, job->n_dpanels, st);
        }
        prof_end(job, st);
    }
    return job_queue_results(job, par, st);
}

int job_run(gauss_job* job, bool solve)
{
    HIPCHK(hipSetDevice(job->ctx->device));
    if (job->run_seq - job->fetch_seq >= 2u)
        return fail(GAUSS_E_INVALID, "gauss_job_run: two runs of this job are in flight already; fetch one first");
    job->prof_run = job->run_seq;
    job->ran_solve = solve;
    const int rc = job_queue_run(job, solve, (int)(job->run_seq & 1u), true);
    if (rc) return rc;
    job->run_seq++;
    job->ran = true;
    return GAUSS_OK;
}


static int ctx_stream_init(gauss_ctx* ctx)
{
    if (ctx->copy) return GAUSS_OK;
    int rc = ctx_stream_create(ctx, &ctx->aux, STREAM_HIGH);
    if (!rc && !ctx->chain) rc = ctx_stream_create(ctx, &ctx->chain, STREAM_HIGH);
    if (rc) return rc;
    HIPCHK(hipStreamCreateWithFlags(&ctx->copy, hipStreamNonBlocking));
    ctx->worker = new CopyWorker(ctx->device);
    return GAUSS_OK;
}

int stream_start_copies(gauss_ctx* ctx, const gauss_window_desc& win, size_t row_bytes, StreamSetup& su)
{
    int rc = ctx_stream_init(ctx);
    if (rc) return rc;
    su.M = win.n_measured; su.U = win.n_unmeasured; su.row_bytes = row_bytes;
    const bool linear = (size_t)win.ld <= row_bytes + row_bytes / 8 + 64;
    su.ldraw = linear ? win.ld : (long long)rup(row_bytes, 16);
    const int ct = 6;
    const int n_ut = (su.U + TILE - 1) / TILE;
    su.tile_group.assign((size_t)std::max(n_ut, 1), 1);
    su.first_tile = {0, 0};
    for (int t = 0, g = 1; t < n_ut; g++) {
        const int sz = std::min(ct, n_ut - t);
        for (int k = 0; k < sz; k++) su.tile_group[(size_t)(t + k)] = g;
        t += sz;
        su.first_tile.push_back(t);
    }
    const int ng = su.n_groups();
    const size_t need = (size_t)(su.M + su.U) * (size_t)su.ldraw + 256;
    if (ctx->landing_bytes < need) {
        if (ctx->landing) { HIPCHK(hipStreamSynchronize(ctx->copy)); HIPCHK(hipFree(ctx->landing)); ctx->landing = nullptr; ctx->landing_bytes = 0; }
        const size_t want = need + need / 4;
        void* d = nullptr;
        hipError_t e = ctx_malloc_retry(ctx, &d, want);
        if (e != hipSuccess) return fail(GAUSS_E_NOMEM, "hipMalloc(%zu bytes landing buffer) failed: %s", want, hipGetErrorString(e));
        ctx->landing = (uint8_t*)d; ctx->landing_bytes = want;
    }
    su.d_m = ctx->landing;
    su.d_u = ctx->landing + rup((size_t)su.M * (size_t)su.ldraw + 64, 256);
    while ((int)ctx->ev_pool.size() < ng) {
        hipEvent_t e;
        HIPCHK(hipEventCreateWithFlags(&e, hipEventDisableTiming));
        ctx->ev_pool.push_back(e);
    }
    su.ev.assign(ctx->ev_pool.begin(), ctx->ev_pool.begin() + ng);
    hipStream_t cs = ctx->copy;
    const uint8_t* hm = win.geno_m;
    const uint8_t* hu = win.geno_u;
    const long long user_ld = win.ld;
    StreamSetup* sp = &su;
    ctx->worker->submit([sp, cs, hm, hu, user_ld, ng]() {
        StreamSetup& su = *sp;
        for (int g = 0; g < ng; g++) {
            const int r0 = g == 0 ? 0 : su.first_tile[(size_t)g] * TILE;
            const int r1 = g == 0 ? su.M : std::min(su.U, su.first_tile[(size_t)g + 1] * TILE);
            const int nrows = r1 - r0;
            uint8_t* dst = (g == 0 ? su.d_m : su.d_u) + (size_t)r0 * su.ldraw;
            const uint8_t* src = (g == 0 ? hm : hu) + (size_t)r0 * user_ld;
            hipError_t e = hipSuccess;
            if (nrows > 0) {
                if (su.ldraw == user_ld)
                    e = hipMemcpyAsync(dst, src, (size_t)(nrows - 1) * user_ld + su.row_bytes, hipMemcpyHostToDevice, cs);
                else
                    e = hipMemcpy2DAsync(dst, (size_t)su.ldraw, src, (size_t)user_ld, su.row_bytes, (size_t)nrows, hipMemcpyHostToDevice, cs);
            }
            if (e == hipSuccess) e = hipEventRecord(su.ev[(size_t)g], cs);
            std::lock_guard<std::mutex> lock(su.mu);
            if (e != hipSuccess) {
                su.rc = GAUSS_E_DEVICE;
                su.err = std::string("streamed window: copy of a chunk failed: ") + hipGetErrorString(e);
                su.recorded = ng;
                su.cv.notify_all();
                return;
            }
            su.recorded = g + 1;
            su.cv.notify_all();
        }
    });
    return GAUSS_OK;
}

int job_run_streamed(gauss_job* job, StreamSetup& su)
{
    gauss_ctx* ctx = job->ctx;
    hipStream_t st = ctx->stream;
    HIPCHK(hipSetDevice(ctx->device));
    hipStream_t ax = ctx->aux;
    hipStream_t ch = ctx->chain;
    Plan& pl = job->plans[0];
    const Prob& p = pl.p;
    const size_t ng = job->sgroups.size();
    const gauss_job::RunEvents& ev = job->rev[job->run_seq & 1u];
    job->queue_touched = true;
    HIPCHK(hipEventRecord(job->begin, st));
    HIPCHK(hipMemsetAsync(job->d_status, 0, sizeof(int) * (4 * job->n + 4), st));
    HIPCHK(hipEventRecord(ev.pack, st));
    HIPCHK(hipStreamWaitEvent(ax, ev.pack, 0));
    for (size_t g = 0; g < ng; g++) {
        const gauss_job::StreamGroup& sg = job->sgroups[g];
        {
            std::unique_lock<std::mutex> lock(su.mu);
            su.cv.wait(lock, [&] { return su.recorded > (int)g; });
            if (su.rc) return fail(su.rc, "%s", su.err.c_str());
        }
        hipStream_t ps = ax;
        HIPCHK(hipStreamWaitEvent(ps, su.ev[g], 0));
        launch_pack_stats(job->d_probs, job->d_rowmap + sg.row0, sg.n_rows, ps);
        if (g == 0) launch_shift_cert(job->d_probs, job->n, ps);
        if (ps != st) {
            HIPCHK(hipEventRecord(job->sevp[g], ps));
            HIPCHK(hipStreamWaitEvent(st, job->sevp[g], 0));
        }
        launch_gram(job->d_items + sg.item0, sg.n_items, job->gram_i8, st);
        if (g == 0) {
            if (ch != st) {
                HIPCHK(hipEventRecord(ev.gram, st));
                HIPCHK(hipStreamWaitEvent(ch, ev.gram, 0));
            }
            launch_epilogue(job->d_probs, job->d_tilemap, job->n_tiles_b11, job->max_pop, job->gram_i8, ch);
            if (pl.out_b11)
                HIPCHK(hipMemcpyAsync(pl.d_b11_copy, p.A, sizeof(double) * p.Mld * p.Mld, hipMemcpyDeviceToDevice, ch));
            for (int s = 0; s < job->max_nblk; s++)
                launch_factor_step(job->d_probs, job->n, s, job->max_nblk, job->max_npanel, job->solve_split, job->own_panel, ch);
            launch_solve_last(job->d_probs, job->d_panelmap, job->n_panels, job->max_nblk, job->solve_split, ch);
            if (ch != st) HIPCHK(hipEventRecord(ev.side, ch));
        }
    }
    launch_epilogue(job->d_probs, job->d_tilemap + job->n_tiles_b11, job->n_tiles - job->n_tiles_b11, job->max_pop, job->gram_i8, st);
    if (ch != st) HIPCHK(hipStreamWaitEvent(st, ev.side, 0));
    launch_loo(job->d_probs, job->d_loomap, job->n_loo, st);
    launch_slct(job->d_probs, job->d_slctmap, job->n_slct, st);
    launch_traits_weights(job->d_probs, job->d_traitsmap, job->n_traits, st);
    launch_impute_gemm(job->d_probs, job->d_gemmmap, job->n_gemm, job->gemm_ut, job->d_finmap, job->n_fin, st);
    launch_traits_impute(job->d_probs, job->d_traitsumap, job->n_traits_u, st);
    const int rc = job_queue_results(job, (int)(job->run_seq & 1u), st);
    if (rc) return rc;
    job->run_seq++;
    job->ran = true;
    job->ran_solve = true;
    return GAUSS_OK;
}

static int job_clamp_window(gauss_job* job, int i, int* status_bits)
{
    hipStream_t st = job->ctx->stream;
    Plan& pl = job->plans[i];
    Prob& p = pl.p;
    std::vector<int2> tm;
    tm = job->win_tiles[(size_t)i];
    DevBuf d_tm, d_work, d_pm, d_lm;
    HIPCHK(d_tm.alloc(job->ctx, sizeof(int2) * tm.size()));
    HIPCHK(hipMemcpyAsync(d_tm.p, tm.data(), sizeof(int2) * tm.size(), hipMemcpyHostToDevice, st));
    launch_epilogue(job->d_probs, d_tm.as<int2>(), (int)tm.size(), job->max_pop, job->gram_i8, st);
    HIPCHK(hipGetLastError());
    const size_t n = (size_t)p.Mld;
    HIPCHK(d_work.alloc(job->ctx, sizeof(double) * (2 * n * n + 4 * n)));
    HIPCHK(hipMemsetAsync(p.status, 0, sizeof(int) * 4, st));
    launch_jacobi_clamp(job->d_probs, i, p, d_work.as<double>(), true, st);
    HIPCHK(hipGetLastError());
    std::vector<int2> pm;
    for (int pn = 0; pn < p.npanel; pn++) pm.push_back(make_int2(i, pn));
    HIPCHK(d_pm.alloc(job->ctx, sizeof(int2) * pm.size()));
    HIPCHK(hipMemcpyAsync(d_pm.p, pm.data(), sizeof(int2) * pm.size(), hipMemcpyHostToDevice, st));
    if (pl.out_b11) HIPCHK(hipMemcpyAsync(pl.d_b11_copy, p.A, sizeof(double) * n * n, hipMemcpyDeviceToDevice, st));
    HIPCHK(hipMemcpyAsync(p.A + 4 * n * n, p.A, sizeof(double) * n * n, hipMemcpyDeviceToDevice, st));
    if (pl.slct_K) launch_slct(job->d_probs + i, nullptr, 1, st);
    const bool loo = pl.loo, traits = pl.traits_T > 0, ride = loo || traits;
    for (int s = 0; s < p.nblk; s++) {
        launch_factor_step(job->d_probs + i, 1, s, p.nblk, ride ? p.npi : 0, ride ? job->solve_split : 0, 0, st);
    }
    const int n_us = (p.U + NB - 1) / NB;
    if (ride) {
        std::vector<int2> lm;
        for (int pn = 0; pn < std::max(p.npi, traits ? n_us : 0); pn++) lm.push_back(make_int2(i, pn));
        const int n_x = (p.M + NR - 1) / NR;
        HIPCHK(d_lm.alloc(job->ctx, sizeof(int2) * lm.size()));
        HIPCHK(hipMemcpyAsync(d_lm.p, lm.data(), sizeof(int2) * lm.size(), hipMemcpyHostToDevice, st));
        launch_solve_last(job->d_probs, d_lm.as<int2>(), p.npi, p.nblk, job->solve_split, st);
// ... 258 lines not shown
```

### gauss_amd/csrc/k_gram.hip

```cpp
#include "gauss_internal.h"
#include "k_gram_common.h"
#include <cstdlib>
#include <type_traits>

#ifndef GAUSS_GRAM_EDGE16
#define GAUSS_GRAM_EDGE16 1
#endif

namespace gauss {

typedef float f32x16 __attribute__((ext_vector_type(16)));
typedef uint32_t u32x4 __attribute__((ext_vector_type(4)));

constexpr int LROW = 64;
constexpr int LTILE = TILE * LROW;

typedef float f32x2 __attribute__((ext_vector_type(2)));

template <int NA, int NB, bool SK10>
__device__ __forceinline__ void chunk_mfma(const uint8_t* __restrict__ la, const uint8_t* __restrict__ lb,
                                           const int (&aoff)[2], const int (&boff)[2], f32x16& acc00, f32x16& acc01,
                                           f32x16& acc10, f32x16& acc11, int nl)
{
#define GAUSS_MFMA_PAIR(AW0, AW1, BW0, BW1, HI)                                                       \
    {                                                                                                  \
        const f32x2 fa0 = __builtin_amdgcn_cvt_pk_f32_fp8((int)(AW0), HI);                             \
        const f32x2 fb0 = __builtin_amdgcn_cvt_pk_f32_fp8((int)(BW0), HI);                             \
        f32x2 fa1 = fa0, fb1 = fb0;                                                                    \
        if (NA > 1) fa1 = __builtin_amdgcn_cvt_pk_f32_fp8((int)(AW1), HI);                             \
        if (NB > 1) fb1 = __builtin_amdgcn_cvt_pk_f32_fp8((int)(BW1), HI);                             \
        _Pragma("unroll") for (int e = 0; e < 2; e++) {                                              \
            acc00 = __builtin_amdgcn_mfma_f32_32x32x2f32(fa0[e], fb0[e], acc00, 0, 0, 0);              \
            if (NB > 1) acc01 = __builtin_amdgcn_mfma_f32_32x32x2f32(fa0[e], fb1[e], acc01, 0, 0, 0);  \
            if (NA > 1) {                                                                              \
                if (!SK10) acc10 = __builtin_amdgcn_mfma_f32_32x32x2f32(fa1[e], fb0[e], acc10, 0, 0, 0); \
                if (NB > 1) acc11 = __builtin_amdgcn_mfma_f32_32x32x2f32(fa1[e], fb1[e], acc11, 0, 0, 0); \
            }                                                                                          \
        }                                                                                              \
    }
#pragma unroll
    for (int g = 0; g < 2; g++) {
        if (4 * g >= nl) break;
        const u32x4 a0 = *reinterpret_cast<const u32x4*>(la + aoff[g]);
        const u32x4 b0 = *reinterpret_cast<const u32x4*>(lb + boff[g]);
        u32x4 a1 = a0, b1 = b0;
        if (NA > 1) a1 = *reinterpret_cast<const u32x4*>(la + aoff[g] + 32 * LROW);
        if (NB > 1) b1 = *reinterpret_cast<const u32x4*>(lb + boff[g] + 32 * LROW);
        const uint32_t aw0[4] = {a0.x, a0.y, a0.z, a0.w};
        const uint32_t aw1[4] = {a1.x, a1.y, a1.z, a1.w};
        const uint32_t bw0[4] = {b0.x, b0.y, b0.z, b0.w};
        const uint32_t bw1[4] = {b1.x, b1.y, b1.z, b1.w};
#pragma unroll
        for (int q = 0; q < 4; q++) {
            if (4 * g + q >= nl) break;
            GAUSS_MFMA_PAIR(aw0[q], aw1[q], bw0[q], bw1[q], false)
            GAUSS_MFMA_PAIR(aw0[q], aw1[q], bw0[q], bw1[q], true)
        }
    }
#undef GAUSS_MFMA_PAIR
}

constexpr int PK_SHIFT = 12;
constexpr int PK_CODE_MAX = 3;
constexpr int PK_F = ((1 << PK_SHIFT) - 1) / (PK_CODE_MAX * PK_CODE_MAX * KC);
static_assert(PK_F == 7 && PK_CODE_MAX * PK_CODE_MAX * KC * PK_F < (1 << PK_SHIFT), "a row's sum between two sub-flushes must stay below 2^PK_SHIFT");
static_assert(2 * PK_SHIFT <= 24, "both rows' sums together must stay an exact f32 integer");

__device__ __forceinline__ float pk_combine(float fa0, float fa1) { return __builtin_fmaf(fa1, (float)(1 << PK_SHIFT), fa0); }

template <int NA, int NB>
__device__ __forceinline__ void chunk_mfma_packed(const uint8_t* __restrict__ la, const uint8_t* __restrict__ lb,
                                                  const int (&aoff)[2], const int (&boff)[2], f32x16& acc0, f32x16& acc1, int nl)
{
#define GAUSS_MFMA_PAIR(AW0, AW1, BW0, BW1, HI)                                                       \
    {                                                                                                  \
        f32x2 fa = __builtin_amdgcn_cvt_pk_f32_fp8((int)(AW0), HI);                                    \
        const f32x2 fb0 = __builtin_amdgcn_cvt_pk_f32_fp8((int)(BW0), HI);                             \
        f32x2 fb1 = fb0;                                                                               \
        if (NA > 1) {                                                                                  \
            const f32x2 fa1 = __builtin_amdgcn_cvt_pk_f32_fp8((int)(AW1), HI);                         \
            fa[0] = pk_combine(fa[0], fa1[0]);                                                         \
            fa[1] = pk_combine(fa[1], fa1[1]);                                                         \
        }                                                                                              \
        if (NB > 1) fb1 = __builtin_amdgcn_cvt_pk_f32_fp8((int)(BW1), HI);                             \
        _Pragma("unroll") for (int e = 0; e < 2; e++) {                                              \
            acc0 = __builtin_amdgcn_mfma_f32_32x32x2f32(fa[e], fb0[e], acc0, 0, 0, 0);                 \
            if (NB > 1) acc1 = __builtin_amdgcn_mfma_f32_32x32x2f32(fa[e], fb1[e], acc1, 0, 0, 0);     \
        }                                                                                              \
    }
#pragma unroll
    for (int g = 0; g < 2; g++) {
        if (4 * g >= nl) break;
        const u32x4 a0 = *reinterpret_cast<const u32x4*>(la + aoff[g]);
        const u32x4 b0 = *reinterpret_cast<const u32x4*>(lb + boff[g]);
        u32x4 a1 = a0, b1 = b0;
        if (NA > 1) a1 = *reinterpret_cast<const u32x4*>(la + aoff[g] + 32 * LROW);
        if (NB > 1) b1 = *reinterpret_cast<const u32x4*>(lb + boff[g] + 32 * LROW);
        const uint32_t aw0[4] = {a0.x, a0.y, a0.z, a0.w};
        const uint32_t aw1[4] = {a1.x, a1.y, a1.z, a1.w};
        const uint32_t bw0[4] = {b0.x, b0.y, b0.z, b0.w};
        const uint32_t bw1[4] = {b1.x, b1.y, b1.z, b1.w};
#pragma unroll
        for (int q = 0; q < 4; q++) {
            if (4 * g + q >= nl) break;
            GAUSS_MFMA_PAIR(aw0[q], aw1[q], bw0[q], bw1[q], false)
            GAUSS_MFMA_PAIR(aw0[q], aw1[q], bw0[q], bw1[q], true)
        }
    }
#undef GAUSS_MFMA_PAIR
}

__device__ __forceinline__ uint32_t pk_sub_flush(float acc, uint32_t run)
{
    const uint32_t u = (uint32_t)acc;
    return run + (u + __umul24(u >> PK_SHIFT, (1u << 16) - (1u << PK_SHIFT)));
}
__device__ __forceinline__ float pk_slab_lo(uint32_t even, uint32_t odd) { return __uint_as_float(__builtin_amdgcn_perm(odd, even, 0x05040100u)); }
__device__ __forceinline__ float pk_slab_hi(uint32_t even, uint32_t odd) { return __uint_as_float(__builtin_amdgcn_perm(odd, even, 0x07060302u)); }

typedef int i32x16 __attribute__((ext_vector_type(16)));
typedef int i32x4 __attribute__((ext_vector_type(4)));

template <int NA, int NB, bool SK10>
__device__ __forceinline__ void chunk_mfma(const uint8_t* __restrict__ la, const uint8_t* __restrict__ lb,
                                           const int (&aoff)[2], const int (&boff)[2], i32x16& acc00, i32x16& acc01,
                                           i32x16& acc10, i32x16& acc11, int nl)
{
#pragma unroll
    for (int g = 0; g < 2; g++) {
        if (4 * g >= nl) break;
        const i32x4 a0 = *reinterpret_cast<const i32x4*>(la + aoff[g]);
        const i32x4 b0 = *reinterpret_cast<const i32x4*>(lb + boff[g]);
        acc00 = __builtin_amdgcn_mfma_i32_32x32x32_i8(a0, b0, acc00, 0, 0, 0);
        if (NB > 1) {
            const i32x4 b1 = *reinterpret_cast<const i32x4*>(lb + boff[g] + 32 * LROW);
            acc01 = __builtin_amdgcn_mfma_i32_32x32x32_i8(a0, b1, acc01, 0, 0, 0);
            if (NA > 1) {
                const i32x4 a1 = *reinterpret_cast<const i32x4*>(la + aoff[g] + 32 * LROW);
                if (!SK10) acc10 = __builtin_amdgcn_mfma_i32_32x32x32_i8(a1, b0, acc10, 0, 0, 0);
                acc11 = __builtin_amdgcn_mfma_i32_32x32x32_i8(a1, b1, acc11, 0, 0, 0);
            }
        } else if (NA > 1) {
            const i32x4 a1 = *reinterpret_cast<const i32x4*>(la + aoff[g] + 32 * LROW);
            acc10 = __builtin_amdgcn_mfma_i32_32x32x32_i8(a1, b0, acc10, 0, 0, 0);
        }
    }
}

// ... 46 lines not shown
                out[(row >> 1) * TILE + col] = slab_pair(slab_u(acce[ga][nc][0]), slab_u(acce[ga][nc][1]));
                out[((row >> 1) + 1) * TILE + col] = slab_pair(slab_u(acce[ga][nc][2]), slab_u(acce[ga][nc][3]));
            } else {
#pragma unroll
                for (int r = 0; r < 4; r++) out[(row + r) * TILE + col] = slab_bits(acce[ga][nc][r]);
            }
        }
}

template <int NA, int NC>
__device__ __forceinline__ void chunk_mfma_edge_packed(const uint8_t* __restrict__ la, const uint8_t* __restrict__ lb, int eoffa,
                                                       int eoffb, f32x4 (&acce)[2][NC])
{
    uint32_t b[NC][4];
#pragma unroll
    for (int nc = 0; nc < NC; nc++) {
        const u32x4 bw = *reinterpret_cast<const u32x4*>(lb + eoffb + nc * 16 * LROW);
        b[nc][0] = bw.x; b[nc][1] = bw.y; b[nc][2] = bw.z; b[nc][3] = bw.w;
    }
#pragma unroll
    for (int ga = 0; ga < 2; ga++) {
        const u32x4 aw = *reinterpret_cast<const u32x4*>(la + eoffa + ga * 16 * LROW);
        u32x4 aw2 = aw;
        if (NA > 1) aw2 = *reinterpret_cast<const u32x4*>(la + eoffa + (ga * 16 + 32) * LROW);
        const uint32_t a[4] = {aw.x, aw.y, aw.z, aw.w};
        const uint32_t a2[4] = {aw2.x, aw2.y, aw2.z, aw2.w};
        if (NC > 1) {
#pragma unroll
            for (int nc = 0; nc < NC; nc++) asm volatile("" : "+v"(b[nc][0]), "+v"(b[nc][1]), "+v"(b[nc][2]), "+v"(b[nc][3]));
        }
#pragma unroll
        for (int w = 0; w < 4; w++) {
#pragma unroll
            for (int hi = 0; hi < 2; hi++) {
                f32x2 fa = hi ? __builtin_amdgcn_cvt_pk_f32_fp8((int)a[w], true) : __builtin_amdgcn_cvt_pk_f32_fp8((int)a[w], false);
                if (NA > 1) {
                    const f32x2 fa2 = hi ? __builtin_amdgcn_cvt_pk_f32_fp8((int)a2[w], true) : __builtin_amdgcn_cvt_pk_f32_fp8((int)a2[w], false);
                    fa[0] = pk_combine(fa[0], fa2[0]);
                    fa[1] = pk_combine(fa[1], fa2[1]);
                }
#pragma unroll
                for (int nc = 0; nc < NC; nc++) {
                    const f32x2 fb = hi ? __builtin_amdgcn_cvt_pk_f32_fp8((int)b[nc][w], true) : __builtin_amdgcn_cvt_pk_f32_fp8((int)b[nc][w], false);
#pragma unroll
                    for (int e = 0; e < 2; e++) acce[ga][nc] = __builtin_amdgcn_mfma_f32_16x16x4f32(fa[e], fb[e], acce[ga][nc], 0, 0, 0);
                }
            }
            __builtin_amdgcn_sched_barrier(0);
        }
    }
}

template <int NA, int NC, typename OUT>
__device__ __forceinline__ void flush_edge_packed(OUT out, int erow0, int ecol0, const uint32_t (&rune)[2][NC][4])
{
#pragma unroll
    for (int ga = 0; ga < 2; ga++)
#pragma unroll
        for (int nc = 0; nc < NC; nc++) {
            const int o = ((erow0 + 16 * ga) >> 1) * TILE + ecol0 + 16 * nc;
            out[o] = pk_slab_lo(rune[ga][nc][0], rune[ga][nc][1]);
            out[o + TILE] = pk_slab_lo(rune[ga][nc][2], rune[ga][nc][3]);
            if (NA > 1) {
                out[o + 16 * TILE] = pk_slab_hi(rune[ga][nc][0], rune[ga][nc][1]);
                out[o + 17 * TILE] = pk_slab_hi(rune[ga][nc][2], rune[ga][nc][3]);
            }
        }
}

template <int N>
__device__ __forceinline__ void wait_dma_barrier()
{
    asm volatile("s_waitcnt vmcnt(%0) lgkmcnt(0)\n\ts_barrier" ::"n"(N) : "memory");
}
template <int NS>
__device__ __forceinline__ void wait_dma_barrier_dyn(int groups_newer)
{
    if (NS <= 2 || groups_newer <= 0) wait_dma_barrier<0>();
    else if (groups_newer == 1) wait_dma_barrier<4>();
    else wait_dma_barrier<8>();
}

template <int NA, int NB, typename ACC, int NS, bool SK10 = false, int NC = 0, bool PK = false>
__device__ __forceinline__ void run_item(const Item& it, uint8_t* lds, int wr, int wc)
{
    const int Kp = it.Kp;
    const auto Ag = it.a;
    const auto Bg = it.b;
    const int tid = threadIdx.x;
    const int lane = tid & 63;
    const int li = lane & 31, lh = lane >> 5;

    const int wave = __builtin_amdgcn_readfirstlane(tid >> 6);
    const int srow = lane >> 2;
    const int spiece = (lane & 3) ^ ((lane >> 4) & 3);
    size_t gsrc[2];
#pragma unroll
    for (int j = 0; j < 2; j++) gsrc[j] = (size_t)(16 * (wave * 2 + j) + srow) * Kp + 16 * spiece;
    typedef __attribute__((address_space(3))) uint8_t* lds_ptr;
    typedef __attribute__((address_space(1))) const uint8_t* glb_ptr;

    ACC acc00 = {0}, acc01 = {0}, acc10 = {0}, acc11 = {0};
    uint32_t run0[16], run1[16];
    if (PK) {
#pragma unroll
        for (int r = 0; r < 16; r++) { run0[r] = 0; run1[r] = 0; }
    }

    const int k0 = it.k0;
    const int nseg = it.nseg;
    const auto seg_k1 = it.seg_k1;
    const auto live_tab = it.chunk_live;
    const int klast = uniform_load<int>(seg_k1, nseg - 1);
    auto out = it.slab;
    const int obase = (wr * 64 + 4 * lh) * TILE + wc * 64 + li;
    const int obase16 = (wr * 32 + 2 * lh) * TILE + wc * 64 + li;

#define GAUSS_STAGE(BUF, KOFF)                                                                                   \
    {                                                                                                            \
        _Pragma("unroll") for (int j = 0; j < 2; j++) {                                                        \
            const int t = wave * 2 + j;                                                                          \
            __builtin_amdgcn_global_load_lds((glb_ptr)Ag + gsrc[j] + (KOFF), (lds_ptr)(lds + (BUF) * 2 * LTILE + t * 1024), 16, 0, 0);          \
            __builtin_amdgcn_global_load_lds((glb_ptr)Bg + gsrc[j] + (KOFF), (lds_ptr)(lds + (BUF) * 2 * LTILE + LTILE + t * 1024), 16, 0, 0);  \
        }                                                                                                        \
    }
    int cur = 0;
    int kpre = k0;
    int ahead = 0;
#pragma unroll
    for (int d = 0; d < NS - 1; d++)
        if (kpre < klast) { GAUSS_STAGE(d, kpre) kpre += KC; ahead++; }
    wait_dma_barrier_dyn<NS>(ahead - 1);
    ahead--;

    const int sw = (li >> 2) & 3;
    int aoff[2], boff[2];
#pragma unroll
    for (int g = 0; g < 2; g++) {
        aoff[g] = (wr * 64 + li) * LROW + 16 * ((2 * g + lh) ^ sw);
        boff[g] = (wc * 64 + li) * LROW + 16 * ((2 * g + lh) ^ sw);
    }

    constexpr bool BE = NC > 0;
    constexpr int NCE = BE ? NC : 1, NGE = PK ? 2 : 4;
    f32x4 acce[NGE][NCE];
    uint32_t rune[2][NCE][4];
    int eoffa = 0, eoffb = 0, erow0 = 0, ecol0 = 0;
    if (BE) {
        const int r16 = lane & 15, q16 = lane >> 4, sw16 = (r16 >> 2) & 3;
#pragma unroll
        for (int ga = 0; ga < NGE; ga++)
#pragma unroll
            for (int nc = 0; nc < NCE; nc++) {
                acce[ga][nc] = f32x4{0.f, 0.f, 0.f, 0.f};
#pragma unroll
                for (int r = 0; r < 4; r++) if (PK) rune[ga & 1][nc][r] = 0;
            }
        eoffa = (wr * 64 + r16) * LROW + 16 * (q16 ^ sw16);
        eoffb = (wc * 64 + r16) * LROW + 16 * (q16 ^ sw16);
        erow0 = wr * 64 + 4 * q16;
        ecol0 = wc * 64 + r16;
    }

    int k = k0;
    uint32_t lbits = uniform_load<uint32_t>(live_tab, k0 >> 9);
    int nl_next = chunk_live_units(lbits, k0 >> 6);
    for (int seg = 0; seg < nseg; seg++) {
        const int kend = uniform_load<int>(seg_k1, seg);
        int since = 0;
        for (; k < kend; k += KC) {
            if (kpre < klast) {
                int nb_ = cur + NS - 1;
                if (nb_ >= NS) nb_ -= NS;
                GAUSS_STAGE(nb_, kpre)
                kpre += KC;
                ahead++;
            }
            const uint8_t* la = lds + cur * 2 * LTILE;
            const uint8_t* lb = la + LTILE;
            const int nl = nl_next;
            if (k + KC < klast) {
                const int c1 = (k + KC) >> 6;
                if ((c1 & 7) == 0) lbits = uniform_load<uint32_t>(live_tab, c1 >> 3);
                nl_next = chunk_live_units(lbits, c1);
            }
            if constexpr (PK) {
                if (NA > 0 && NB > 0) chunk_mfma_packed<NA, (NB > 0 ? NB : 1)>(la, lb, aoff, boff, acc00, acc01, nl);
                if (BE) chunk_mfma_edge_packed<(NA > 0 ? NA : 1), NCE>(la, lb, eoffa, eoffb, acce);
                if (++since == PK_F || k + KC >= kend) {
                    since = 0;
                    if (NA > 0 && NB > 0) {
#pragma unroll
                        for (int r = 0; r < 16; r++) {
                            run0[r] = pk_sub_flush(acc00[r], run0[r]); acc00[r] = 0;
                            if (NB > 1) { run1[r] = pk_sub_flush(acc01[r], run1[r]); acc01[r] = 0; }
                        }
                    }
                    if (BE) {
#pragma unroll
                        for (int ga = 0; ga < 2; ga++)
#pragma unroll
                            for (int nc = 0; nc < NCE; nc++)
#pragma unroll
                                for (int r = 0; r < 4; r++) { rune[ga][nc][r] = pk_sub_flush(acce[ga][nc][r], rune[ga][nc][r]); acce[ga][nc][r] = 0.f; }
                    }
                }
            } else {
                if (NA > 0 && NB > 0) chunk_mfma<NA, (NB > 0 ? NB : 1), SK10>(la, lb, aoff, boff, acc00, acc01, acc10, acc11, nl);
                if (BE) chunk_mfma_edge<(NA > 0 ? NA : 1), NCE>(la, lb, eoffa, eoffb, acce);
            }
            wait_dma_barrier_dyn<NS>(ahead - 1);
            if (ahead > 0) ahead--;
            cur = (cur + 1 == NS) ? 0 : cur + 1;
        }
#undef GAUSS_STAGE
        if constexpr (PK) {
            if (NA > 0 && NB > 0) {
                int ob = obase16;
                asm volatile("" : "+v"(ob));
#pragma unroll
                for (int r = 0; r < 16; r += 2) {
                    const int o = ob + (((r & 3) + 8 * (r >> 2)) >> 1) * TILE;
                    out[o] = pk_slab_lo(run0[r], run0[r + 1]);
                    if (NB > 1) out[o + 32] = pk_slab_lo(run1[r], run1[r + 1]);
                    if (NA > 1) {
                        out[o + 16 * TILE] = pk_slab_hi(run0[r], run0[r + 1]);
                        if (NB > 1) out[o + 16 * TILE + 32] = pk_slab_hi(run1[r], run1[r + 1]);
                    }
                }
#pragma unroll
                for (int r = 0; r < 16; r++) { run0[r] = 0; run1[r] = 0; }
            }
            if (BE) {
                int er = erow0, ec = ecol0;
                asm volatile("" : "+v"(er), "+v"(ec));
                flush_edge_packed<(NA > 0 ? NA : 1), NCE>(out, er, ec, rune);
#pragma unroll
                for (int ga = 0; ga < 2; ga++)
#pragma unroll
                    for (int nc = 0; nc < NCE; nc++)
#pragma unroll
                        for (int r = 0; r < 4; r++) rune[ga][nc][r] = 0;
            }
            out += TILE * TILE / 2;
        } else {
            if (NA > 0 && NB > 0) {
                int ob = obase, ob16 = obase16;
                asm volatile("" : "+v"(ob), "+v"(ob16));
                flush_acc<NA, (NB > 0 ? NB : 1), SK10>(out, (it.flags & 2) != 0, ob, ob16, acc00, acc01, acc10, acc11);
#pragma unroll
                for (int r = 0; r < 16; r++) { acc00[r] = 0; acc01[r] = 0; acc10[r] = 0; acc11[r] = 0; }
            }
            if (BE) {
                int er = erow0, ec = ecol0;
                asm volatile("" : "+v"(er), "+v"(ec));
                flush_edge<(NA > 0 ? NA : 1), NCE>(out, (it.flags & 2) != 0, er, ec, acce);
#pragma unroll
                for (int ga = 0; ga < 4; ga++)
#pragma unroll
                    for (int nc = 0; nc < NCE; nc++) acce[ga][nc] = f32x4{0.f, 0.f, 0.f, 0.f};
            }
            out += (it.flags & 2) ? TILE * TILE / 2 : TILE * TILE;
        }
    }
}

template <typename ACC, int NS>
__device__ __forceinline__ void gram_item(const Item& it, uint8_t* lds)
{
    const int wave = __builtin_amdgcn_readfirstlane(threadIdx.x >> 6);
    const int wr = wave >> 1, wc = wave & 1;

    int na = (it.rows_a - wr * 64 + 31) / 32;
    int nb = (it.rows_b - wc * 64 + 31) / 32;
    na = na < 0 ? 0 : (na > 2 ? 2 : na);
    nb = nb < 0 ? 0 : (nb > 2 ? 2 : nb);
    const bool diag = (it.flags & 1) != 0;
    if (diag && wr == 1 && wc == 0) na = 0;
    int nc = 0;
    if (std::is_same<ACC, f32x16>::value && GAUSS_GRAM_EDGE16 && na > 0) {
        int nb16 = (it.rows_b - wc * 64 + 15) / 16;
        nb16 = nb16 < 0 ? 0 : (nb16 > 4 ? 4 : nb16);
        if (nb16 & 1) nc = nb16;
    }
    if constexpr (std::is_same<ACC, f32x16>::value) {
        if (it.flags & 4) {
            if (nc == 3) { if (na == 2) run_item<2, 0, ACC, NS, false, 3, true>(it, lds, wr, wc); else run_item<1, 0, ACC, NS, false, 3, true>(it, lds, wr, wc); }
            else if (nc == 1) { if (na == 2) run_item<2, 0, ACC, NS, false, 1, true>(it, lds, wr, wc); else run_item<1, 0, ACC, NS, false, 1, true>(it, lds, wr, wc); }
            else if (na == 0 || nb == 0) run_item<0, 0, ACC, NS>(it, lds, wr, wc);
            else if (na == 2 && nb == 2) run_item<2, 2, ACC, NS, false, 0, true>(it, lds, wr, wc);
            else if (na == 2) run_item<2, 1, ACC, NS, false, 0, true>(it, lds, wr, wc);
            else if (nb == 2) run_item<1, 2, ACC, NS, false, 0, true>(it, lds, wr, wc);
            else run_item<1, 1, ACC, NS, false, 0, true>(it, lds, wr, wc);
            return;
        }
    }
    if (nc == 3) { if (na == 2) run_item<2, 0, ACC, NS, false, 3>(it, lds, wr, wc); else run_item<1, 0, ACC, NS, false, 3>(it, lds, wr, wc); return; }
    if (nc == 1) { if (na == 2) run_item<2, 0, ACC, NS, false, 1>(it, lds, wr, wc); else run_item<1, 0, ACC, NS, false, 1>(it, lds, wr, wc); return; }
    if (na == 0 || nb == 0) run_item<0, 0, ACC, NS>(it, lds, wr, wc);
    else if (na == 2 && nb == 2 && diag && wr == wc) run_item<2, 2, ACC, NS, true>(it, lds, wr, wc);
    else if (na == 2 && nb == 2) run_item<2, 2, ACC, NS>(it, lds, wr, wc);
    else if (na == 2) run_item<2, 1, ACC, NS>(it, lds, wr, wc);
    else if (nb == 2) run_item<1, 2, ACC, NS>(it, lds, wr, wc);
    else run_item<1, 1, ACC, NS>(it, lds, wr, wc);
}

template <typename ACC, int NS, int OCC>
__global__ __launch_bounds__(256, OCC) __attribute__((amdgpu_num_vgpr(52))) void gram_kernel(const Item* __restrict__ items,
                                                                                             unsigned long long* __restrict__ b11_done)
{
    __shared__ __attribute__((aligned(16))) uint8_t lds[NS * 2 * LTILE];

    const Item& it = items[blockIdx.x];
    const int counted = it.flags & 48;
    gram_item<ACC, NS>(it, lds);
    if (counted && b11_done) {
        asm volatile("s_waitcnt vmcnt(0)" ::: "memory");
        __syncthreads();
        if (threadIdx.x == 0) {
            __builtin_amdgcn_fence(__ATOMIC_RELEASE, "agent");
            asm volatile("s_waitcnt vmcnt(0)" ::: "memory");
            __hip_atomic_fetch_add(b11_done + ((counted & 32) ? 8 : 0), 1ull, __ATOMIC_RELAXED, __HIP_MEMORY_SCOPE_AGENT);
        }
    }
}

__global__ __launch_bounds__(64) void wait_count_kernel(const unsigned long long* __restrict__ count, unsigned long long target,
                                                        unsigned long long timeout_ticks, int* __restrict__ status, int n_status)
{
    if (threadIdx.x != 0) return;
    __builtin_amdgcn_s_setprio(3);
    const unsigned long long t0 = wall_clock64();
    for (;;) {
        if (__hip_atomic_load(count, __ATOMIC_RELAXED, __HIP_MEMORY_SCOPE_AGENT) >= target) return;
        if (wall_clock64() - t0 > timeout_ticks) break;
        __builtin_amdgcn_s_sleep(127);
    }
    for (int i = 0; i < n_status; i++) status[i] = 1;
}

__global__ __launch_bounds__(64) void count_up_kernel(unsigned long long* __restrict__ count)
{
    if (threadIdx.x == 0) __hip_atomic_fetch_add(count, 1ull, __ATOMIC_RELEASE, __HIP_MEMORY_SCOPE_AGENT);
}

void launch_count_up(unsigned long long* d_count, hipStream_t s)
{
    hipLaunchKernelGGL(count_up_kernel, dim3(1), dim3(64), 0, s, d_count);
}

void launch_wait_count_for(const unsigned long long* d_count, unsigned long long target, int* d_status, hipStream_t s, double bound_us)
{
    hipLaunchKernelGGL(wait_count_kernel, dim3(1), dim3(64), 0, s, d_count, target, (unsigned long long)(bound_us * 100.0), d_status, 1);
}

void launch_wait_count(const unsigned long long* d_count, unsigned long long target, int* d_status, int n_status, hipStream_t s,
                       double bound_us)
{
    unsigned long long ticks = bound_us > 2e6 ? (unsigned long long)(bound_us * 100.0) : 200000000ull;
    if (const char* e = getenv("GAUSS_WAIT_COUNT_TIMEOUT_US")) {
        const long long us = atoll(e);
        if (us < 0) target = ~0ull;
        ticks = (unsigned long long)(us < 0 ? -us : us) * 100ull;
    }
    hipLaunchKernelGGL(wait_count_kernel, dim3(1), dim3(64), 0, s, d_count, target, ticks, d_status, n_status);
}

void launch_gram(const Item* d_items, int n_items, int dtype_i8, hipStream_t s, unsigned long long* d_b11_done)
{
    if (n_items <= 0) return;
#ifndef GAUSS_I8_NS
#define GAUSS_I8_NS 2
#define GAUSS_I8_OCC 4
#endif
    if (dtype_i8) hipLaunchKernelGGL((gram_kernel<i32x16, GAUSS_I8_NS, GAUSS_I8_OCC>), dim3(n_items), dim3(256), 0, s, d_items, d_b11_done);
    else hipLaunchKernelGGL((gram_kernel<f32x16, 2, 4>), dim3(n_items), dim3(256), 0, s, d_items, d_b11_done);
}

}
```

### gauss_amd/csrc/k_pack_epilogue.hip

```cpp
#include "gauss_internal.h"

namespace gauss {

struct __attribute__((packed)) U32u { uint32_t v; };

__global__ __launch_bounds__(256) void pack_stats_kernel(const Prob* __restrict__ probs,
                                                         const int2* __restrict__ rowmap)
{
    __shared__ int s_sx[64];
    __shared__ int s_sxx[64];
    constexpr int PACK_LDS_WORDS = 8192;
    __shared__ uint8_t s_word[PACK_LDS_WORDS];
    __shared__ int s_pk[65], s_src[65], s_len[64];
    __shared__ double s_cov[64], s_mm[64], s_wmu[64];
    const int2 rm = rowmap[blockIdx.x];
    const Prob& pb = probs[rm.x];
    const int r = rm.y;
    const uint8_t* src;
    int prow;
    const bool um = r >= pb.M;
    int code = 0;
    if (!um) {
        const long long srow = pb.rows_m ? pb.rows_m[r] : r;
        src = pb.raw_m + (size_t)srow * pb.ld_raw; prow = r;
    } else {
        const int ur = r - pb.M;
        const int blk = ur / pb.U_raw;
        const int rr = ur - blk * pb.U_raw;
        const long long srow = pb.rows_u ? pb.rows_u[rr] : rr;
        src = pb.raw_u + (size_t)srow * pb.ld_raw;
        prow = ur;
        code = pb.code_blk[blk];
    }
    uint4* dst = reinterpret_cast<uint4*>((um ? pb.packed_u : pb.packed) + (size_t)prow * pb.Kp);

    if (threadIdx.x < 64) { s_sx[threadIdx.x] = 0; s_sxx[threadIdx.x] = 0; }
    const int nwords = pb.Kp >> 4;
    const bool fmt2 = pb.geno_fmt != 0;
    const int n_tab = fmt2 ? pb.n_run : pb.P;
    const bool tab_lds = nwords <= PACK_LDS_WORDS;
    {
        const auto wt = fmt2 ? pb.word_run : pb.word_pop;
        if (tab_lds)
            for (int w = threadIdx.x; w < nwords; w += 256) s_word[w] = wt[w];
        if (threadIdx.x < n_tab) {
            const int r = threadIdx.x;
            s_pk[r] = fmt2 ? pb.run_pk_off[r] : pb.pop_pk_off[r];
            s_src[r] = fmt2 ? pb.run_src[r] : pb.pop_raw_off[r];
            s_len[r] = fmt2 ? 0 : pb.pop_raw_off[r + 1] - pb.pop_raw_off[r];
        }
    }
    __syncthreads();

    auto finish_word = [&](int w, bool live, int p, uint32_t (&v)[4]) {
        int sx = 0, sxx = 0;
#pragma unroll
        for (int q = 0; q < 4; q++) {
            uint32_t x = fmt2 ? v[q] : (v[q] & 0x0F0F0F0Fu);
            if (code) {
                const uint32_t ge4 = ((x >> 2) | (x >> 3)) & 0x01010101u;
                const uint32_t is3 = x & (x >> 1) & 0x01010101u & ~ge4;
                const uint32_t keep = (ge4 | is3) * 0xFFu;
                const uint32_t rec = (code == 1) ? ((x | (x >> 1)) & 0x01010101u) : ((x >> 1) & 0x01010101u);
                x = (x & keep) | (rec & ~keep);
            }
            sx = __builtin_amdgcn_udot4(x, 0x01010101u, sx, false);
            sxx = __builtin_amdgcn_udot4(x, x, sxx, false);
            uint32_t c;
            if (pb.gram_i8) {
                c = x;
            } else if (fmt2 || (x & 0x08080808u) == 0) {
                c = __builtin_amdgcn_perm(0x4E4C4A48u, 0x44403800u, x);
            } else {
                c = 0;
#pragma unroll
                for (int b = 0; b < 4; b++) {
                    const uint32_t t = (x >> (8 * b)) & 0xFu;
                    const uint32_t e = t == 0 ? 0u : t == 1 ? 0x38u : t < 4 ? 0x40u + 4u * (t - 2) : t < 8 ? 0x48u + 2u * (t - 4) : 0x50u + (t - 8);
                    c |= e << (8 * b);
                }
            }
            v[q] = c;
        }
        {
            const bool odd = (w & 1) != 0;
            const uint32_t s0 = odd ? v[0] : v[1], s1 = odd ? v[2] : v[3];
            const uint32_t r0 = (uint32_t)__builtin_amdgcn_update_dpp(0, (int)s0, 0xB1, 0xF, 0xF, true);
            const uint32_t r1 = (uint32_t)__builtin_amdgcn_update_dpp(0, (int)s1, 0xB1, 0xF, 0xF, true);
            if (live) dst[w] = odd ? make_uint4(r0, r1, v[1], v[3]) : make_uint4(v[0], v[2], r0, r1);
        }
        sx += __builtin_amdgcn_update_dpp(0, sx, 0xB1, 0xF, 0xF, true);
        sxx += __builtin_amdgcn_update_dpp(0, sxx, 0xB1, 0xF, 0xF, true);
        sx += __builtin_amdgcn_update_dpp(0, sx, 0x4E, 0xF, 0xF, true);
        sxx += __builtin_amdgcn_update_dpp(0, sxx, 0x4E, 0xF, 0xF, true);
        if ((threadIdx.x & 3) == 0 && sx) { atomicAdd(&s_sx[p], sx); atomicAdd(&s_sxx[p], sxx); }
    };

    const int nloop = (nwords + 255) & ~255;
    if (fmt2 && tab_lds) {
#ifndef GAUSS_PACK_BATCH
#define GAUSS_PACK_BATCH 4
#endif
        constexpr int PB = GAUSS_PACK_BATCH;
        for (int w0 = threadIdx.x; w0 < nloop; w0 += PB * 256) {
            uint32_t bits[PB];
            int ww[PB], pp[PB];
            bool lv[PB];
#pragma unroll
            for (int j = 0; j < PB; j++) {
                const int wj = w0 + 256 * j;
                lv[j] = wj < nwords;
                ww[j] = lv[j] ? wj : nwords - 1;
                const int run = s_word[ww[j]];
                pp[j] = (pb.P == 1) ? 0 : run;
                const int o = (ww[j] << 4) - s_pk[run];
                bits[j] = lv[j] ? *reinterpret_cast<const uint32_t*>(src + s_src[run] + (o >> 2)) : 0u;
            }
#pragma unroll
            for (int j = 0; j < PB; j++) {
                if (w0 + 256 * j >= nloop) break;
                uint32_t v[4];
#pragma unroll
                for (int q = 0; q < 4; q++) {
                    uint32_t b = (bits[j] >> (8 * q)) & 0xFFu;
                    b = (b | (b << 12)) & 0x000F000Fu;
                    v[q] = (b | (b << 6)) & 0x03030303u;
                }
                finish_word(ww[j], lv[j], pp[j], v);
            }
        }
    } else {
        for (int w0 = threadIdx.x; w0 < nloop; w0 += 256) {
            const bool live = w0 < nwords;
            const int w = live ? w0 : nwords - 1;
            const int run = tab_lds ? s_word[w] : (fmt2 ? pb.word_run[w] : pb.word_pop[w]);
            const int p = (pb.P == 1) ? 0 : run;
            const int o = (w << 4) - s_pk[run];
            uint32_t v[4] = {0u, 0u, 0u, 0u};
            if (fmt2) {
                const uint32_t bits = live ? *reinterpret_cast<const uint32_t*>(src + s_src[run] + (o >> 2)) : 0u;
#pragma unroll
                for (int q = 0; q < 4; q++) {
                    uint32_t b = (bits >> (8 * q)) & 0xFFu;
                    b = (b | (b << 12)) & 0x000F000Fu;
                    v[q] = (b | (b << 6)) & 0x03030303u;
                }
            } else {
                int valid = s_len[run] - o;
                valid = valid < 0 ? 0 : (valid > 16 ? 16 : valid);
                if (!live) valid = 0;
                const uint8_t* s = src + s_src[run] + o;
                if (valid == 16) {
#pragma unroll
                    for (int q = 0; q < 4; q++) v[q] = reinterpret_cast<const U32u*>(s + 4 * q)->v;
                } else {
                    for (int b = 0; b < valid; b++) v[b >> 2] |= (uint32_t)s[b] << (8 * (b & 3));
                }
            }
            finish_word(w, live, p, v);
        }
    }
    __syncthreads();
    const int P = pb.P;
    if (threadIdx.x < P) {
        (um ? pb.sx_u : pb.sx)[(size_t)prow * P + threadIdx.x] = s_sx[threadIdx.x];
        (um ? pb.sxx_u : pb.sxx)[(size_t)prow * P + threadIdx.x] = s_sxx[threadIdx.x];
    }
    const auto rt_wm = um ? pb.rt_wm_u : pb.rt_wm;
    const auto rt_sd = um ? pb.rt_sd_u : pb.rt_sd;
    if (pb.mode == 0) {
        if (threadIdx.x == 0) {
            double sumx = 0, sumxsq = 0;
            int num_samples = 0;
            for (int p = 0; p < P; p++) {
                sumx += (double)s_sx[p];
                sumxsq += (double)s_sxx[p];
                num_samples += pb.pop_raw_off[p + 1] - pb.pop_raw_off[p];
            }
            rt_wm[prow] = sumx;
            rt_sd[prow] = sqrt((num_samples) * sumxsq - sumx * sumx);
        }
        return;
    }
    if (threadIdx.x < P) {
        const int p = threadIdx.x;
        const int m = pb.pop_raw_off[p + 1] - pb.pop_raw_off[p];
        const double wgt_val = pb.pop_w[p];
        const double sumx = (double)s_sx[p];
        const double sumxy = (double)s_sxx[p];
        const double factor = ((double)m) / (m - 1);
        s_cov[p] = wgt_val * factor * (m * sumxy - sumx * sumx);
        const double mu = sumx / m;
        const double wmu = wgt_val * mu;
        s_mm[p] = wmu * mu;
        s_wmu[p] = wmu;
        (um ? pb.rt_mu_u : pb.rt_mu)[(size_t)prow * P + p] = mu;
        (um ? pb.rt_wmu_u : pb.rt_wmu)[(size_t)prow * P + p] = wmu;
    }
    __syncthreads();
    if (threadIdx.x == 0) {
        double wsumcov = 0, wsum_mi_mj = 0, wsum_mi = 0;
        for (int p = 0; p < P; p++) { wsumcov += s_cov[p]; wsum_mi_mj += s_mm[p]; wsum_mi += s_wmu[p]; }
        rt_wm[prow] = wsum_mi;
        rt_sd[prow] = sqrt(wsumcov + wsum_mi_mj - wsum_mi * wsum_mi);
    }
}

void launch_pack_stats(const Prob* d_probs, const int2* d_rowmap, int n_rows, hipStream_t s)
{
    if (n_rows > 0) hipLaunchKernelGGL(pack_stats_kernel, dim3(n_rows), dim3(256), 0, s, d_probs, d_rowmap);
}

__device__ __forceinline__ double slab_val(float v, int is_int) { return is_int ? (double)__float_as_int(v) : (double)v; }

__device__ __forceinline__ double cor_entry(const Prob& pb, const float* __restrict__ tile_slab,
                                            int off, int ri, int rj, bool ri_unmeasured = false)
{
    const int P = pb.P;
    const auto rt_wm_i = ri_unmeasured ? pb.rt_wm_u : pb.rt_wm;
    const auto rt_sd_i = ri_unmeasured ? pb.rt_sd_u : pb.rt_sd;
    const size_t seg_stride = (size_t)TILE * TILE;
    if (pb.mode == 0) {
        double sumxy = 0;
        for (int s = 0; s < pb.nseg; s++) sumxy += slab_val(tile_slab[s * seg_stride + off], pb.gram_i8);
        const int num_samples = pb.N;
        const double numer = num_samples * sumxy - rt_wm_i[ri] * pb.rt_wm[rj];
        const double denor = rt_sd_i[ri] * pb.rt_sd[rj];
        return numer / denor;
    }
    double wsumcov = 0, wsum_mi_mj = 0;
    const int* sxi = (ri_unmeasured ? pb.sx_u : pb.sx) + (size_t)ri * P;
    const int* sxj = pb.sx + (size_t)rj * P;
    const double* wmui = (ri_unmeasured ? pb.rt_wmu_u : pb.rt_wmu) + (size_t)ri * P;
    const double* muj = pb.rt_mu + (size_t)rj * P;
    for (int p = 0; p < P; p++) {
        double sumxy = 0;
        for (int s = pb.pop_seg0[p]; s < pb.pop_seg0[p + 1]; s++)
            sumxy += slab_val(tile_slab[s * seg_stride + off], pb.gram_i8);
        const double sumx = (double)sxi[p], sumy = (double)sxj[p];
        wsumcov += pb.pop_wf[p] * (pb.pop_md[p] * sumxy - sumx * sumy);
        wsum_mi_mj += wmui[p] * muj[p];
    }
    const double cov = wsumcov + wsum_mi_mj - rt_wm_i[ri] * pb.rt_wm[rj];
    return cov / (rt_sd_i[ri] * pb.rt_sd[rj]);
}
// ... 540 lines not shown
```

### gauss_amd/hotpath.py

```python
import ctypes as C

import numpy as np

from . import _lib
from ._lib import MODE_POOLED, MODE_WEIGHTED, WindowDesc, check

_dp = C.POINTER(C.c_double)
_ip = C.POINTER(C.c_int32)


class Context:

    def __init__(self, device=0):
        self.lib = _lib.load()
        h = C.c_void_p()
        check(self.lib.gauss_hip_init(int(device), C.byref(h)))
        self.handle = h
        self.device = device

    def set_gram_dtype(self, dtype):
        code = {"f32": _lib.GRAM_F32, "i8": _lib.GRAM_I8}[dtype] if isinstance(dtype, str) else int(dtype)
        check(self.lib.gauss_hip_set_gram_dtype(self.handle, code))

    @property
# ... 403 lines not shown
            self._host = rows
            check(self.ctx.lib.gauss_store_alloc(self.ctx.handle, rows.nbytes, C.byref(p)))
        elif asynchronous:
            self._host = rows
            check(self.ctx.lib.gauss_store_upload_async(self.ctx.handle, rows.ctypes.data_as(C.c_void_p), rows.nbytes, C.byref(p)))
        else:
            check(self.ctx.lib.gauss_store_upload(self.ctx.handle, rows.ctypes.data_as(C.c_void_p), rows.nbytes, C.byref(p)))
        self.ptr = p.value

    def fill(self, r0, r1):
        if self._fd is not None:
            check(self.ctx.lib.gauss_store_fill_fd(self.ctx.handle, C.c_void_p(self.ptr), self._fd, C.c_int64(self._file_off),
                                                   C.c_int64(int(r0) * self.ld), C.c_int64((int(r1) - int(r0)) * self.ld)))
            return
        check(self.ctx.lib.gauss_store_fill(self.ctx.handle, C.c_void_p(self.ptr), self._host.ctypes.data_as(C.c_void_p),
                                            int(r0) * self.ld, (int(r1) - int(r0)) * self.ld))

    def wait(self, n_rows=0):
        check(self.ctx.lib.gauss_store_wait(self.ctx.handle, C.c_void_p(self.ptr), int(n_rows) * self.ld))

    def close(self):
        if self.ptr:
            self.ctx.lib.gauss_store_free(self.ctx.handle, C.c_void_p(self.ptr))
            self.ptr = None
        if getattr(self, "_fd", None) is not None:
            import os
            os.close(self._fd)
            self._fd = None

    def __del__(self):
        try:
            self.close()
        except Exception:
            pass


class Job:

    def __init__(self, windows, ctx=None, on_device=False, want_mats=False):
        self.ctx = ctx or default_context()
        n = len(windows)
        self.descs = (WindowDesc * n)()
        self.wins = []
        for i, w in enumerate(windows):
            self.wins.append(_Win(self.descs[i], w["mode"], w.get("geno_m"), w.get("geno_u"),
                                  w["pop_off"], w.get("pop_wgt"), w["z1"], w.get("lam", 0.1),
                                  w.get("min_abs_eig", 1e-5), want_mats, w.get("dev"), w.get("qcat"), w.get("ld_codings"), w.get("packed"),
                                  loo=bool(w.get("loo", False)), slct=w.get("slct"), z_more=w.get("z_more")))
        h = C.c_void_p()
        check(self.ctx.lib.gauss_job_create(self.ctx.handle, self.descs, n, 1 if on_device else 0,
                                            C.byref(h)))
        self.handle = h

    def run(self):
        check(self.ctx.lib.gauss_job_run(self.handle))

    def fetch(self):
        check(self.ctx.lib.gauss_job_fetch(self.handle))
        return [w.result() for w in self.wins]

    def counters(self):
        out = (C.c_int64 * 4)()
        check(self.ctx.lib.gauss_job_counters(self.handle, out))
        return dict(merged=int(out[0]), demoted=int(out[1]), giveups=int(out[2]), rerun_failed=int(out[3]))

    def profile(self, enable=True):
        check(self.ctx.lib.gauss_job_profile(self.handle, 1 if enable else 0))

    def profile_get(self, kernel=0):
        ms, n = C.c_double(), C.c_int64()
        check(self.ctx.lib.gauss_job_profile_get(self.handle, kernel, C.byref(ms), C.byref(n)))
        return ms.value, n.value

    def work(self):
        a, b, c, d = C.c_double(), C.c_double(), C.c_double(), C.c_int64()
        check(self.ctx.lib.gauss_job_work(self.handle, C.byref(a), C.byref(b), C.byref(c), C.byref(d)))
        return dict(ld_flops=a.value, solve_flops=b.value, bytes=c.value, imputed_snps=d.value)

    def stats(self):
        out = (C.c_double * 4)()
        check(self.ctx.lib.gauss_job_stats(self.handle, out))
        return dict(items=int(out[0]), executed_flops=out[1], slab_bytes=out[2], workspace_bytes=out[3])

    def close(self):
        if self.handle:
            self.ctx.lib.gauss_job_destroy(self.handle)
            self.handle = None

    def __del__(self):
        try:
            self.close()
        except Exception:
            pass
```

### include/gauss_hip.h

```cpp
#ifndef GAUSS_HIP_H
#define GAUSS_HIP_H

#include <stddef.h>
#include <stdint.h>

#ifdef __cplusplus
extern "C" {
#endif

#define GAUSS_MODE_POOLED   0
#define GAUSS_MODE_WEIGHTED 1

#define GAUSS_OK            0
#define GAUSS_E_INVALID    -1
#define GAUSS_E_DEVICE     -2
#define GAUSS_E_NOMEM      -3
#define GAUSS_E_RANGE      -4

#define GAUSS_ST_CLAMPED    1
#define GAUSS_ST_NONFINITE  2
#define GAUSS_ST_NOCONV     4
#define GAUSS_ST_SLCT_SKIPPED 8

typedef struct gauss_ctx gauss_ctx;
// ... 67 lines not shown
int gauss_store_upload(gauss_ctx* ctx, const void* host_rows, int64_t bytes, void** out_device_ptr);
int gauss_store_upload_fd(gauss_ctx* ctx, int fd, int64_t file_offset, int64_t bytes, void** out_device_ptr);
int gauss_store_free(gauss_ctx* ctx, void* device_ptr);
int gauss_store_alloc(gauss_ctx* ctx, int64_t bytes, void** out_device_ptr);
int gauss_store_fill(gauss_ctx* ctx, void* device_ptr, const void* host_rows, int64_t offset, int64_t len);
int gauss_store_fill_fd(gauss_ctx* ctx, void* device_ptr, int fd, int64_t file_offset, int64_t offset, int64_t len);
int gauss_store_upload_async(gauss_ctx* ctx, const void* host_rows, int64_t bytes, void** out_device_ptr);
int gauss_store_upload_fd_async(gauss_ctx* ctx, int fd, int64_t file_offset, int64_t bytes, void** out_device_ptr);
int gauss_store_wait(gauss_ctx* ctx, const void* device_ptr, int64_t bytes_needed);

int gauss_hip_init(int device, gauss_ctx** out_ctx);
int gauss_hip_device_count(int* out_n);
int gauss_hip_device_of(const gauss_ctx* ctx);
void gauss_hip_destroy(gauss_ctx* ctx);
uint64_t gauss_hip_context_id(const gauss_ctx* ctx);
int gauss_hip_add_destroy_hook(void (*fn)(gauss_ctx* ctx, uint64_t id, void* user), void* user);
int gauss_hip_trim_cache(gauss_ctx* ctx, int64_t* out_bytes_freed);
int gauss_hip_counters(gauss_ctx* ctx, int64_t* out4);
int gauss_job_counters(gauss_job* job, int64_t* out4);
int gauss_hip_queues(gauss_ctx* ctx, int32_t* out4);
const char* gauss_last_error(void);
const char* gauss_hip_version(void);
const char* gauss_hip_source_hash(void);

#define GAUSS_GRAM_F32 0
#define GAUSS_GRAM_I8  1
int gauss_hip_set_gram_dtype(gauss_ctx* ctx, int dtype);


int gauss_ld(gauss_ctx* ctx, int mode, const uint8_t* geno, int n_snp, int64_t ld,
             const int32_t* pop_off, const double* pop_wgt, int n_pop, double diag,
             double* out_cor);

int gauss_impute_window(gauss_ctx* ctx, const gauss_window_desc* win);

int gauss_gene_ld_batch(gauss_ctx* ctx, int mode, const uint8_t* geno, int n_snp, int64_t ld,
                        const int32_t* pop_off, const double* pop_wgt, int n_pop,
                        const int32_t* gene_off, int n_gene, double diag, double* out_blocks);

int gauss_ld_rows(gauss_ctx* ctx, int mode, const uint8_t* store, int64_t ld, int geno_format, const int32_t* rows, int n_snp,
                  const int32_t* pop_off, const int32_t* pop_src_off, const double* pop_wgt, int n_pop, double diag,
                  int on_device, double* out_cor);
int gauss_gene_ld_batch_rows(gauss_ctx* ctx, int mode, const uint8_t* store, int64_t ld, int geno_format, const int32_t* rows,
                             int n_snp, const int32_t* pop_off, const int32_t* pop_src_off, const double* pop_wgt, int n_pop,
                             const int32_t* gene_off, int n_gene, double diag, int on_device, double* out_blocks);

int gauss_ld_resampled_rows(gauss_ctx* ctx, const uint8_t* store, int64_t ld, int geno_format, const int32_t* rows, int n_snp,
                            const int32_t* pop_off, const int32_t* pop_src_off, int n_pop,
                            const int32_t* draw_pop, const int32_t* draw_sample, int64_t n_drawn, int64_t n_cols,
                            double diag, int on_device, double* out_cor);

int gauss_ld_per_pop(gauss_ctx* ctx, const uint8_t* geno, int n_snp, int64_t ld,
                     const int32_t* pop_off, int n_pop, double* out);

int gauss_ld_per_pop_pairs(gauss_ctx* ctx, const uint8_t* geno, int n_snp, int64_t ld, const int32_t* pop_off, int n_pop,
                           const int32_t* pop_group, int n_group, const int32_t* pair_i, const int32_t* pair_j, int64_t n_pairs,
                           double* out);

int gauss_pop_weights(gauss_ctx* ctx, const double* x, const int64_t* interval_off, int n_interval, int n_pop,
                      double min_abs_eig, double* out_w_interval, int32_t* out_status);

int gauss_zmix_normal_eq(gauss_ctx* ctx, const uint8_t* geno, int n_snp, int64_t ld, const int32_t* pop_off, int n_pop,
                         const int32_t* pop_group, int n_group, const double* z, double* out_xtx, double* out_xty, double* out_yty,
                         int64_t* out_n_rows);

int gauss_gram_counts(gauss_ctx* ctx, const uint8_t* geno, int n_snp, int n_samples, int64_t ld,
                      int64_t* out_counts);


int gauss_job_create(gauss_ctx* ctx, const gauss_window_desc* wins, int n_win, int on_device,
                     gauss_job** out_job);
int gauss_job_run(gauss_job* job);
int gauss_job_fetch(gauss_job* job);
void gauss_job_destroy(gauss_job* job);
int gauss_job_span_ms(gauss_job* first, gauss_job* last, double* out_ms);

int gauss_job_profile(gauss_job* job, int enable);
int gauss_job_profile_get(gauss_job* job, int kernel, double* out_ms, int64_t* out_launches);
int gauss_job_work(gauss_job* job, double* out_ld_flops, double* out_solve_flops,
                   double* out_bytes, int64_t* out_imputed_snps);

int gauss_job_stats(gauss_job* job, double* out4);

int gauss_pack2bit_device(gauss_ctx* ctx, const uint8_t* d_in, int64_t ld_in, uint8_t* d_out, int64_t ld_out,
                          int n_snp, const int32_t* pop_off, int n_pop);

int gauss_synth_device(gauss_ctx* ctx, uint8_t* d_out, int n_snp, int64_t ld,
                       const int32_t* pop_off, int n_pop, const float* thr, const float* rho,
                       uint64_t seed);

#ifdef __cplusplus
}
#endif
#endif
```

Baseline: 3.725 million.

## Adapt packed-Gram sub-flush interval per tile based on presence of code-3 genotypes

```diff
diff --git a/gauss_amd/_lib.py b/gauss_amd/_lib.py
--- a/gauss_amd/_lib.py
+++ b/gauss_amd/_lib.py
@@ -55,7 +55,7 @@
     "gauss_hip_init", "gauss_hip_device_count", "gauss_hip_device_of", "gauss_hip_destroy", "gauss_last_error", "gauss_hip_version", "gauss_hip_set_gram_dtype", "gauss_pinned_alloc", "gauss_pinned_free", "gauss_store_upload", "gauss_store_free", "gauss_pack2bit_device", "gauss_ld", "gauss_ld_per_pop", "gauss_ld_per_pop_pairs",
     "gauss_impute_window", "gauss_gene_ld_batch", "gauss_gram_counts", "gauss_job_create",
     "gauss_ld_rows", "gauss_gene_ld_batch_rows", "gauss_job_run", "gauss_job_fetch", "gauss_job_destroy", "gauss_job_span_ms", "gauss_job_profile",
-    "gauss_job_profile_get", "gauss_job_work", "gauss_job_stats", "gauss_synth_device",
+    "gauss_job_profile_get", "gauss_job_work", "gauss_job_stats", "gauss_job_code3_tiles", "gauss_synth_device",
     "gauss_store_upload_async", "gauss_store_upload_fd_async", "gauss_store_wait", "gauss_store_alloc", "gauss_store_fill", "gauss_store_fill_fd", "gauss_store_upload_fd", "gauss_hip_context_id", "gauss_hip_add_destroy_hook", "gauss_hip_trim_cache", "gauss_hip_source_hash", "gauss_hip_counters", "gauss_job_counters", "gauss_hip_queues",
     "gauss_pop_weights", "gauss_zmix_normal_eq", "gauss_ld_resampled_rows",
 ]
@@ -118,6 +118,7 @@
     lib.gauss_job_counters.argtypes = [C.c_void_p, C.POINTER(C.c_int64)]
     lib.gauss_job_work.argtypes = [C.c_void_p, _dp, _dp, _dp, C.POINTER(C.c_int64)]
     lib.gauss_job_stats.argtypes = [C.c_void_p, _dp]
+    lib.gauss_job_code3_tiles.argtypes = [C.c_void_p, C.POINTER(C.c_uint32), C.c_int, C.POINTER(C.c_int)]
     lib.gauss_hip_context_id.argtypes = [C.c_void_p]
     lib.gauss_hip_context_id.restype = C.c_uint64
     lib.gauss_hip_trim_cache.argtypes = [C.c_void_p, C.POINTER(C.c_int64)]
diff --git a/gauss_amd/csrc/gauss_abi.cpp b/gauss_amd/csrc/gauss_abi.cpp
--- a/gauss_amd/csrc/gauss_abi.cpp
+++ b/gauss_amd/csrc/gauss_abi.cpp
@@ -108,6 +108,19 @@
 {
     if (!job || !out4) return fail(GAUSS_E_INVALID, "bad arguments to gauss_job_counters");
     out4[0] = job->n_merged; out4[1] = job->n_demoted; out4[2] = job->n_giveups; out4[3] = job->n_rerun_failed;
+    return GAUSS_OK;
+}
+
+int gauss_job_code3_tiles(gauss_job* job, uint32_t* out, int cap, int* out_n)
+{
+    if (!job || !out_n || (cap > 0 && !out)) return fail(GAUSS_E_INVALID, "bad arguments");
+    *out_n = job->d_tile3 ? job->n_tile3 : 0;
+    const int n = std::min(*out_n, cap);
+    if (n <= 0) return GAUSS_OK;
+    if (!job->ctx) return fail(GAUSS_E_INVALID, "the job's context is gone");
+    HIPCHK(hipSetDevice(job->ctx->device));
+    HIPCHK(hipStreamSynchronize(job->ctx->stream));
+    HIPCHK(hipMemcpy(out, job->d_tile3, sizeof(uint32_t) * (size_t)n, hipMemcpyDeviceToHost));
     return GAUSS_OK;
 }
 
diff --git a/gauss_amd/csrc/gauss_ctx.cpp b/gauss_amd/csrc/gauss_ctx.cpp
--- a/gauss_amd/csrc/gauss_ctx.cpp
+++ b/gauss_amd/csrc/gauss_ctx.cpp
@@ -211,6 +211,7 @@
     const char* e = getenv("GAUSS_GRAM_DTYPE");
     c->gram_i8 = (e && (strcmp(e, "i8") == 0 || strcmp(e, "int8") == 0)) ? 1 : 0;
     c->gram_packed = env_int("GAUSS_GRAM_PACKED", 1) != 0 ? 1 : 0;
+    c->gram_subflush_adapt = env_int("GAUSS_GRAM_SUBFLUSH_ADAPT", 1) != 0 ? 1 : 0;
     const char* one = getenv("GAUSS_SIDE_STREAM");
     c->main_cls = (one && atoi(one) == 0) ? STREAM_NORMAL : STREAM_HIGH;
     int rc = ctx_stream_create(c, &c->stream, c->main_cls);
diff --git a/gauss_amd/csrc/gauss_internal.h b/gauss_amd/csrc/gauss_internal.h
--- a/gauss_amd/csrc/gauss_internal.h
+++ b/gauss_amd/csrc/gauss_internal.h
@@ -72,6 +72,8 @@
     GP(const int) run_pk_off;
     GP(const int) run_src;
     GP(float) slab;
+    GP(uint32_t) tile3;
+    GP(uint32_t) tile3_u;
     GP(double) rt_sd;
     GP(double) rt_wm;
     GP(double) rt_mu;
@@ -171,7 +173,8 @@
 constexpr int SIMLD_LDS_MAX = 60 << 10;
 int resample_pack_lds_bytes(long long row_src_bytes);
 void launch_resample_pack(const Prob* d_probs, const int2* d_rowmap, int n_rows, int lds_bytes, hipStream_t s);
-void launch_gram(const Item* d_items, int n_items, int dtype_i8, hipStream_t s, unsigned long long* d_b11_done = nullptr);
+void launch_gram(const Item* d_items, int n_items, int dtype_i8, hipStream_t s, unsigned long long* d_b11_done = nullptr,
+                 const uint32_t* d_tile3 = nullptr);
 void launch_wait_count(const unsigned long long* d_count, unsigned long long target, int* d_status, int n_status, hipStream_t s,
                        double bound_us = 0.0);
 void launch_wait_count_for(const unsigned long long* d_count, unsigned long long target, int* d_status, hipStream_t s, double bound_us);
diff --git a/gauss_amd/csrc/gauss_job.h b/gauss_amd/csrc/gauss_job.h
--- a/gauss_amd/csrc/gauss_job.h
+++ b/gauss_amd/csrc/gauss_job.h
@@ -139,6 +139,7 @@
     std::map<const void*, std::shared_ptr<StoreUpload>> uploads;
     int gram_i8 = 0;
     int gram_packed = 1;
+    int gram_subflush_adapt = 1;
     std::map<const void*, size_t> stores;
     std::mutex mu;
     BlockCache dev_cache, pin_cache;
@@ -283,6 +284,9 @@
     int max_pop = 1;
     int gram_i8 = 0;
     int gram_packed = 0;
+    int subflush_adapt = 0;
+    int n_tile3 = 0;
+    uint32_t* d_tile3 = nullptr;
     int resample_lds = -1;
     int* d_status = nullptr;
     unsigned long long* d_b11_done = nullptr;
diff --git a/gauss_amd/csrc/gauss_plan.cpp b/gauss_amd/csrc/gauss_plan.cpp
--- a/gauss_amd/csrc/gauss_plan.cpp
+++ b/gauss_amd/csrc/gauss_plan.cpp
@@ -325,6 +325,7 @@
     job->on_device = on_device;
     job->gram_i8 = ctx->gram_i8;
     job->gram_packed = (ctx->gram_packed && !ctx->gram_i8) ? 1 : 0;
+    job->subflush_adapt = (job->gram_packed && ctx->gram_subflush_adapt && !streamed) ? 1 : 0;
     job->plans.resize(job->n);
     for (const WinSpec& w : specs)
         if (w.draw_pop && (specs.size() != 1 || streamed)) return fail(GAUSS_E_INVALID, "a resampled window is a job of its own");
@@ -803,7 +804,20 @@
         go.wmu = wa.take(rows * q.P * sizeof(double));
         go.slab = wslab.take((size_t)q.npair * q.nseg * TILE * TILE * (q.slab16 ? sizeof(uint16_t) : sizeof(float)));
     }
-    const size_t o_status = wa.take(sizeof(int) * (4 * job->n + 4));
+    std::vector<int> t3_m((size_t)job->n, 0), t3_u((size_t)job->n, 0);
+    int n_tile3 = 0;
+    if (job->subflush_adapt) {
+        if (shm && job->gplan->p.slab16) n_tile3 += job->gplan->p.nT + 2;
+        for (int i = 0; i < job->n; i++) {
+            const Prob& p = job->plans[i].p;
+            if (!p.slab16 || !job->plans[i].draw_col.empty()) continue;
+            t3_m[(size_t)i] = n_tile3; n_tile3 += p.Mp / TILE;
+            t3_u[(size_t)i] = n_tile3; n_tile3 += p.Up / TILE;
+        }
+        if (n_tile3 >= (1 << 22)) { n_tile3 = 0; job->subflush_adapt = 0; }
+    }
+    job->n_tile3 = n_tile3;
+    const size_t o_status = wa.take(sizeof(int) * (4 * job->n + 4 + (size_t)n_tile3));
     const size_t o_count = wa.take(128);
     const size_t o_results = wa.take(sizeof(double) * std::max<size_t>(res, 1));
     job->n_results = res;
@@ -871,6 +885,7 @@
     }
 
     job->d_status = (int*)(job->d_ws + o_status);
+    job->d_tile3 = n_tile3 ? (uint32_t*)(job->d_status + 4 * job->n + 4) : nullptr;
     job->d_b11_done = (unsigned long long*)(job->d_ws + o_count);
     job->d_results = (double*)(job->d_ws + o_results);
     std::deque<std::vector<uint8_t>> stage;
@@ -934,6 +949,9 @@
         p.rt_sd_u = p.rt_sd + p.Mp; p.rt_wm_u = p.rt_wm + p.Mp;
         p.rt_mu_u = p.rt_mu + (size_t)p.Mp * p.P; p.rt_wmu_u = p.rt_wmu + (size_t)p.Mp * p.P;
         p.g0 = 0; p.n_gpair = 0; p.gpair_ti = p.pair_ti; p.gpair_tj = p.pair_tj; p.slab_g = p.slab;
+        const bool t3 = job->d_tile3 && p.slab16 && pl.draw_col.empty();
+        p.tile3 = (t3 && !shm) ? job->d_tile3 + t3_m[(size_t)i] : nullptr;
+        p.tile3_u = t3 ? job->d_tile3 + t3_u[(size_t)i] : nullptr;
         if (shm) {
             const Prob& q = job->gplan->p;
             const size_t g0 = (size_t)job->g0[(size_t)i];
@@ -990,6 +1008,7 @@
         q.word_pop = (const uint8_t*)(T + to[n].wp); q.word_run = (const uint8_t*)(T + to[n].wr);
         q.rows_m = (const int*)(T + to[n].rm); q.rows_u = nullptr;
         q.run_pk_off = (const int*)(T + to[n].rpk); q.run_src = (const int*)(T + to[n].rsrc);
+        q.tile3 = (job->d_tile3 && q.slab16) ? job->d_tile3 : nullptr; q.tile3_u = q.tile3;
         q.slab = (float*)(W + go.slab); q.slab_g = q.slab; q.gpair_ti = q.pair_ti; q.gpair_tj = q.pair_tj; q.g0 = 0; q.n_gpair = q.npair;
         q.z1 = nullptr; q.A = nullptr; q.B21 = nullptr; q.Linv = nullptr; q.V = nullptr; q.Gsum = nullptr; q.Part = nullptr;
         q.out_z = q.out_info = nullptr; q.out_loo = nullptr; q.out_slct = nullptr; q.slct_W = nullptr; q.slct_forced = nullptr; q.slct_max = 0; q.traits_T = 0; q.traits_Z = nullptr; q.traits_Y = q.traits_G = q.out_traits = nullptr; q.out_ld = nullptr; q.status = job->d_status;
@@ -1015,7 +1034,21 @@
         it.seg_k1 = p.seg_k1 + gr.first;
         it.chunk_live = (const uint32_t*)(job->d_tab + to[h.prob].ch);
         it.Kp = p.Kp; it.k0 = pl.seg_k0[gr.first]; it.nseg = gr.second - gr.first;
-        it.rows_a = rows(ti); it.rows_b = rows(tj); it.flags = (ti == tj ? 1 : 0) | (p.slab16 ? 2 : 0) | (p.slab16 && job->gram_packed ? 4 : 0);
+        it.rows_a = rows(ti); it.rows_b = rows(tj);
+        int two_a = 0, two_b = 0;
+        if (job->d_tile3 && p.slab16 && job->gram_packed && pl.draw_col.empty()) {
+            auto t3_word = [&](int t, int& two) {
+                if (t >= mt) return t3_u[(size_t)h.prob] + (t - mt) + 1;
+                if ((int)h.prob == job->n) return t + 1;
+                if (!shm) return t3_m[(size_t)h.prob] + t + 1;
+                const int r0 = p.g0 + t * TILE;
+                two = (r0 % TILE) != 0;
+                return r0 / TILE + 1;
+            };
+            it.rows_a |= t3_word(ti, two_a) << 8;
+            it.rows_b |= t3_word(tj, two_b) << 8;
+        }
+        it.flags = (two_a ? 64 : 0) | (two_b ? 128 : 0) | (ti == tj ? 1 : 0) | (p.slab16 ? 2 : 0) | (p.slab16 && job->gram_packed ? 4 : 0);
         if (job->merged && (int)n < job->n_items_b11) it.flags |= 16;
         else if (job->merged && (int)n < job->n_items_b11 + job->n_items_b21_early) it.flags |= 32;
         memcpy(blob.data() + o_items + sizeof(Item) * n, &it, sizeof(Item));
diff --git a/gauss_amd/csrc/gauss_run.cpp b/gauss_amd/csrc/gauss_run.cpp
--- a/gauss_amd/csrc/gauss_run.cpp
+++ b/gauss_amd/csrc/gauss_run.cpp
@@ -73,7 +73,7 @@
     if (job->merged && solve) { (merged ? ctx->n_runs_merged : ctx->n_runs_demoted)++; (merged ? job->n_merged : job->n_demoted)++; }
     const auto t_run0 = std::chrono::steady_clock::now();
     HIPCHK(hipEventRecord(job->begin, st));
-    HIPCHK(hipMemsetAsync(job->d_status, 0, sizeof(int) * (4 * job->n + 4), st));
+    HIPCHK(hipMemsetAsync(job->d_status, 0, sizeof(int) * (4 * job->n + 4 + (size_t)job->n_tile3), st));
     if (trace_on("job")) fprintf(stderr, "[job] run (%s): begin mark + status zeroing queued in %.2f ms\n", merged ? "merged" : (job->chain_aside ? "two launches" : "one queue"),
                                  std::chrono::duration<double, std::milli>(std::chrono::steady_clock::now() - t_run0).count());
     const bool fused = env_int("GAUSS_FUSED_SOLVE", 1) != 0 || job->n_loo > 0 || job->n_traits > 0;
@@ -89,7 +89,7 @@
         if (merged) {
             HIPCHK(hipEventRecord(ev.gram, st));
             prof_begin(job, 0, st, 1);
-            launch_gram(job->d_items, job->n_items, job->gram_i8, st, job->d_b11_done);
+            launch_gram(job->d_items, job->n_items, job->gram_i8, st, job->d_b11_done, job->d_tile3);
             job->merged_runs++;
             prof_end(job, st);
             HIPCHK(hipStreamWaitEvent(ch, ev.gram, 0));
@@ -97,9 +97,9 @@
             launch_wait_count(job->d_b11_done, job->merged_runs * (unsigned long long)job->n_items_b11, job->d_status + 4 * job->n, 1, ch, job->wait_bound_us);
         } else {
             prof_begin(job, 0, st, 2);
-            launch_gram(job->d_items, job->n_items_b11, job->gram_i8, st);
+            launch_gram(job->d_items, job->n_items_b11, job->gram_i8, st, nullptr, job->d_tile3);
             HIPCHK(hipEventRecord(ev.gram, st));
-            launch_gram(job->d_items + job->n_items_b11, job->n_items - job->n_items_b11, job->gram_i8, st);
+            launch_gram(job->d_items + job->n_items_b11, job->n_items - job->n_items_b11, job->gram_i8, st, nullptr, job->d_tile3);
             prof_end(job, st);
             HIPCHK(hipStreamWaitEvent(ch, ev.gram, 0));
         }
@@ -144,7 +144,7 @@
         return job_queue_results(job, par, st);
     }
     prof_begin(job, 0, st, 1);
-    launch_gram(job->d_items, job->n_items, job->gram_i8, st);
+    launch_gram(job->d_items, job->n_items, job->gram_i8, st, nullptr, job->d_tile3);
     prof_end(job, st);
     if (side) {
         HIPCHK(hipEventRecord(ev.gram, st));
@@ -296,7 +296,7 @@
     const gauss_job::RunEvents& ev = job->rev[job->run_seq & 1u];
     job->queue_touched = true;
     HIPCHK(hipEventRecord(job->begin, st));
-    HIPCHK(hipMemsetAsync(job->d_status, 0, sizeof(int) * (4 * job->n + 4), st));
+    HIPCHK(hipMemsetAsync(job->d_status, 0, sizeof(int) * (4 * job->n + 4 + (size_t)job->n_tile3), st));
     HIPCHK(hipEventRecord(ev.pack, st));
     HIPCHK(hipStreamWaitEvent(ax, ev.pack, 0));
     for (size_t g = 0; g < ng; g++) {
diff --git a/gauss_amd/csrc/k_gram.hip b/gauss_amd/csrc/k_gram.hip
--- a/gauss_amd/csrc/k_gram.hip
+++ b/gauss_amd/csrc/k_gram.hip
@@ -62,8 +62,12 @@
 
 constexpr int PK_SHIFT = 12;
 constexpr int PK_CODE_MAX = 3;
+constexpr int pk_interval(int amax, int bmax) { return ((1 << PK_SHIFT) - 1) / (amax * bmax * KC); }
 constexpr int PK_F = ((1 << PK_SHIFT) - 1) / (PK_CODE_MAX * PK_CODE_MAX * KC);
 static_assert(PK_F == 7 && PK_CODE_MAX * PK_CODE_MAX * KC * PK_F < (1 << PK_SHIFT), "a row's sum between two sub-flushes must stay below 2^PK_SHIFT");
+static_assert(PK_F == pk_interval(PK_CODE_MAX, PK_CODE_MAX), "the same rule");
+static_assert(pk_interval(2, 2) == 15 && 2 * 2 * KC * pk_interval(2, 2) < (1 << PK_SHIFT), "no code 3 in either tile");
+static_assert(pk_interval(3, 2) == 10 && pk_interval(2, 3) == 10 && 3 * 2 * KC * pk_interval(3, 2) < (1 << PK_SHIFT), "a code 3 in one tile");
 static_assert(2 * PK_SHIFT <= 24, "both rows' sums together must stay an exact f32 integer");
 
 __device__ __forceinline__ float pk_combine(float fa0, float fa1) { return __builtin_fmaf(fa1, (float)(1 << PK_SHIFT), fa0); }
@@ -276,7 +280,7 @@
 }
 
 template <int NA, int NB, typename ACC, int NS, bool SK10 = false, int NC = 0, bool PK = false>
-__device__ __forceinline__ void run_item(const Item& it, uint8_t* lds, int wr, int wc)
+__device__ __forceinline__ void run_item(const Item& it, uint8_t* lds, int wr, int wc, GP(const uint32_t) tile3 = nullptr)
 {
     const int Kp = it.Kp;
     const auto Ag = it.a;
@@ -306,6 +310,16 @@
     const auto seg_k1 = it.seg_k1;
     const auto live_tab = it.chunk_live;
     const int klast = uniform_load<int>(seg_k1, nseg - 1);
+    int pk_f = PK_F;
+    if constexpr (PK) {
+        const int ta = it.rows_a >> 8, tb = it.rows_b >> 8;
+        if (tile3 && ta && tb) {
+            uint32_t a3 = uniform_load<uint32_t>(tile3, ta - 1), b3 = uniform_load<uint32_t>(tile3, tb - 1);
+            if (it.flags & 64) a3 |= uniform_load<uint32_t>(tile3, ta);
+            if (it.flags & 128) b3 |= uniform_load<uint32_t>(tile3, tb);
+            pk_f = a3 ? (b3 ? pk_interval(3, 3) : pk_interval(3, 2)) : (b3 ? pk_interval(2, 3) : pk_interval(2, 2));
+        }
+    }
     auto out = it.slab;
     const int obase = (wr * 64 + 4 * lh) * TILE + wc * 64 + li;
     const int obase16 = (wr * 32 + 2 * lh) * TILE + wc * 64 + li;
@@ -381,7 +395,7 @@
             if constexpr (PK) {
                 if (NA > 0 && NB > 0) chunk_mfma_packed<NA, (NB > 0 ? NB : 1)>(la, lb, aoff, boff, acc00, acc01, nl);
                 if (BE) chunk_mfma_edge_packed<(NA > 0 ? NA : 1), NCE>(la, lb, eoffa, eoffb, acce);
-                if (++since == PK_F || k + KC >= kend) {
+                if (++since == pk_f || k + KC >= kend) {
                     since = 0;
                     if (NA > 0 && NB > 0) {
 #pragma unroll
@@ -460,32 +474,33 @@
 }
 
 template <typename ACC, int NS>
-__device__ __forceinline__ void gram_item(const Item& it, uint8_t* lds)
+__device__ __forceinline__ void gram_item(const Item& it, uint8_t* lds, GP(const uint32_t) tile3)
 {
     const int wave = __builtin_amdgcn_readfirstlane(threadIdx.x >> 6);
     const int wr = wave >> 1, wc = wave & 1;
 
-    int na = (it.rows_a - wr * 64 + 31) / 32;
-    int nb = (it.rows_b - wc * 64 + 31) / 32;
+    const int rows_a = it.rows_a & 255, rows_b = it.rows_b & 255;
+    int na = (rows_a - wr * 64 + 31) / 32;
+    int nb = (rows_b - wc * 64 + 31) / 32;
     na = na < 0 ? 0 : (na > 2 ? 2 : na);
     nb = nb < 0 ? 0 : (nb > 2 ? 2 : nb);
     const bool diag = (it.flags & 1) != 0;
     if (diag && wr == 1 && wc == 0) na = 0;
     int nc = 0;
     if (std::is_same<ACC, f32x16>::value && GAUSS_GRAM_EDGE16 && na > 0) {
-        int nb16 = (it.rows_b - wc * 64 + 15) / 16;
+        int nb16 = (rows_b - wc * 64 + 15) / 16;
         nb16 = nb16 < 0 ? 0 : (nb16 > 4 ? 4 : nb16);
         if (nb16 & 1) nc = nb16;
     }
     if constexpr (std::is_same<ACC, f32x16>::value) {
         if (it.flags & 4) {
-            if (nc == 3) { if (na == 2) run_item<2, 0, ACC, NS, false, 3, true>(it, lds, wr, wc); else run_item<1, 0, ACC, NS, false, 3, true>(it, lds, wr, wc); }
-            else if (nc == 1) { if (na == 2) run_item<2, 0, ACC, NS, false, 1, true>(it, lds, wr, wc); else run_item<1, 0, ACC, NS, false, 1, true>(it, lds, wr, wc); }
+            if (nc == 3) { if (na == 2) run_item<2, 0, ACC, NS, false, 3, true>(it, lds, wr, wc, tile3); else run_item<1, 0, ACC, NS, false, 3, true>(it, lds, wr, wc, tile3); }
+            else if (nc == 1) { if (na == 2) run_item<2, 0, ACC, NS, false, 1, true>(it, lds, wr, wc, tile3); else run_item<1, 0, ACC, NS, false, 1, true>(it, lds, wr, wc, tile3); }
             else if (na == 0 || nb == 0) run_item<0, 0, ACC, NS>(it, lds, wr, wc);
-            else if (na == 2 && nb == 2) run_item<2, 2, ACC, NS, false, 0, true>(it, lds, wr, wc);
-            else if (na == 2) run_item<2, 1, ACC, NS, false, 0, true>(it, lds, wr, wc);
-            else if (nb == 2) run_item<1, 2, ACC, NS, false, 0, true>(it, lds, wr, wc);
-            else run_item<1, 1, ACC, NS, false, 0, true>(it, lds, wr, wc);
+            else if (na == 2 && nb == 2) run_item<2, 2, ACC, NS, false, 0, true>(it, lds, wr, wc, tile3);
+            else if (na == 2) run_item<2, 1, ACC, NS, false, 0, true>(it, lds, wr, wc, tile3);
+            else if (nb == 2) run_item<1, 2, ACC, NS, false, 0, true>(it, lds, wr, wc, tile3);
+            else run_item<1, 1, ACC, NS, false, 0, true>(it, lds, wr, wc, tile3);
             return;
         }
     }
@@ -501,13 +516,14 @@
 
 template <typename ACC, int NS, int OCC>
 __global__ __launch_bounds__(256, OCC) __attribute__((amdgpu_num_vgpr(52))) void gram_kernel(const Item* __restrict__ items,
-                                                                                             unsigned long long* __restrict__ b11_done)
+                                                                                             unsigned long long* __restrict__ b11_done,
+                                                                                             const uint32_t* __restrict__ tile3)
 {
     __shared__ __attribute__((aligned(16))) uint8_t lds[NS * 2 * LTILE];
 
     const Item& it = items[blockIdx.x];
     const int counted = it.flags & 48;
-    gram_item<ACC, NS>(it, lds);
+    gram_item<ACC, NS>(it, lds, (GP(const uint32_t))tile3);
     if (counted && b11_done) {
         asm volatile("s_waitcnt vmcnt(0)" ::: "memory");
         __syncthreads();
@@ -560,15 +576,15 @@
     hipLaunchKernelGGL(wait_count_kernel, dim3(1), dim3(64), 0, s, d_count, target, ticks, d_status, n_status);
 }
 
-void launch_gram(const Item* d_items, int n_items, int dtype_i8, hipStream_t s, unsigned long long* d_b11_done)
+void launch_gram(const Item* d_items, int n_items, int dtype_i8, hipStream_t s, unsigned long long* d_b11_done, const uint32_t* d_tile3)
 {
     if (n_items <= 0) return;
 #ifndef GAUSS_I8_NS
 #define GAUSS_I8_NS 2
 #define GAUSS_I8_OCC 4
 #endif
-    if (dtype_i8) hipLaunchKernelGGL((gram_kernel<i32x16, GAUSS_I8_NS, GAUSS_I8_OCC>), dim3(n_items), dim3(256), 0, s, d_items, d_b11_done);
-    else hipLaunchKernelGGL((gram_kernel<f32x16, 2, 4>), dim3(n_items), dim3(256), 0, s, d_items, d_b11_done);
-}
-
-}
+    if (dtype_i8) hipLaunchKernelGGL((gram_kernel<i32x16, GAUSS_I8_NS, GAUSS_I8_OCC>), dim3(n_items), dim3(256), 0, s, d_items, d_b11_done, d_tile3);
+    else hipLaunchKernelGGL((gram_kernel<f32x16, 2, 4>), dim3(n_items), dim3(256), 0, s, d_items, d_b11_done, d_tile3);
+}
+
+}
diff --git a/gauss_amd/csrc/k_pack_epilogue.hip b/gauss_amd/csrc/k_pack_epilogue.hip
--- a/gauss_amd/csrc/k_pack_epilogue.hip
+++ b/gauss_amd/csrc/k_pack_epilogue.hip
@@ -34,6 +34,9 @@
     }
     uint4* dst = reinterpret_cast<uint4*>((um ? pb.packed_u : pb.packed) + (size_t)prow * pb.Kp);
 
+    __shared__ int s_has3;
+    if (threadIdx.x == 0) s_has3 = 0;
+    uint32_t has3 = 0;
     if (threadIdx.x < 64) { s_sx[threadIdx.x] = 0; s_sxx[threadIdx.x] = 0; }
     const int nwords = pb.Kp >> 4;
     const bool fmt2 = pb.geno_fmt != 0;
@@ -115,6 +118,7 @@
                 pp[j] = (pb.P == 1) ? 0 : run;
                 const int o = (ww[j] << 4) - s_pk[run];
                 bits[j] = lv[j] ? *reinterpret_cast<const uint32_t*>(src + s_src[run] + (o >> 2)) : 0u;
+                has3 |= bits[j] & (bits[j] >> 1);
             }
 #pragma unroll
             for (int j = 0; j < PB; j++) {
@@ -139,6 +143,7 @@
             uint32_t v[4] = {0u, 0u, 0u, 0u};
             if (fmt2) {
                 const uint32_t bits = live ? *reinterpret_cast<const uint32_t*>(src + s_src[run] + (o >> 2)) : 0u;
+                has3 |= bits & (bits >> 1);
 #pragma unroll
                 for (int q = 0; q < 4; q++) {
                     uint32_t b = (bits >> (8 * q)) & 0xFFu;
@@ -160,7 +165,10 @@
             finish_word(w, live, p, v);
         }
     }
+    const auto tile3 = um ? pb.tile3_u : pb.tile3;
+    if (tile3 && (has3 & 0x55555555u)) s_has3 = 1;
     __syncthreads();
+    if (tile3 && threadIdx.x == 0 && s_has3) atomicOr(&tile3[prow / TILE], 1u);
     const int P = pb.P;
     if (threadIdx.x < P) {
         (um ? pb.sx_u : pb.sx)[(size_t)prow * P + threadIdx.x] = s_sx[threadIdx.x];
diff --git a/gauss_amd/hotpath.py b/gauss_amd/hotpath.py
--- a/gauss_amd/hotpath.py
+++ b/gauss_amd/hotpath.py
@@ -509,6 +509,13 @@
         check(self.ctx.lib.gauss_job_stats(self.handle, out))
         return dict(items=int(out[0]), executed_flops=out[1], slab_bytes=out[2], workspace_bytes=out[3])
 
+    def code3_tiles(self):
+        n = C.c_int()
+        check(self.ctx.lib.gauss_job_code3_tiles(self.handle, None, 0, C.byref(n)))
+        out = np.zeros(max(n.value, 1), dtype=np.uint32)
+        check(self.ctx.lib.gauss_job_code3_tiles(self.handle, out.ctypes.data_as(C.POINTER(C.c_uint32)), n.value, C.byref(n)))
+        return out[:n.value]
+
     def close(self):
         if self.handle:
             self.ctx.lib.gauss_job_destroy(self.handle)
diff --git a/include/gauss_hip.h b/include/gauss_hip.h
--- a/include/gauss_hip.h
+++ b/include/gauss_hip.h
@@ -173,6 +173,8 @@
 
 int gauss_job_stats(gauss_job* job, double* out4);
 
+int gauss_job_code3_tiles(gauss_job* job, uint32_t* out, int cap, int* out_n);
+
 int gauss_pack2bit_device(gauss_ctx* ctx, const uint8_t* d_in, int64_t ld_in, uint8_t* d_out, int64_t ld_out,
                           int n_snp, const int32_t* pop_off, int n_pop);
 
```

Result: no change. 3.750 million (median of 6 runs) (+0.7%).
